# s-esposito/MonoGS

Measured on AMD Instinct MI355X. Metric: rasteriser fwd+bwd Mpix/s @1080p, higher is better.
Workload: dtype f32; 1 GPU; C5: 2000000 Gaussians, 1920x1080, fwd+bwd, seeded synthetic map (SURVEY.md 8d), one keyframe per GPU; gaussians=2000000, width=1920, height=1080, settle_steps=60, instance_count=device-side (capacity mode, overflow checked), parallelism=keyframe-per-gpu x1

## Files before the change

### monogs_amd/csrc/api.hip

```cpp
#include "common.h"

#include <stdarg.h>
#include <stdio.h>
#include <string.h>

namespace mgs {

static thread_local char g_err[512] = "";

void set_error(const char* fmt, ...) {
    va_list ap;
    va_start(ap, fmt);
    vsnprintf(g_err, sizeof(g_err), fmt, ap);
    va_end(ap);
}

static inline char* take(char*& p, size_t bytes) {
    char* r = p;
    p += align_up(bytes, 256);
    return r;
}

GeometryState GeometryState::carve(void* base, int P) {
    char* p = (char*)align_up((size_t)base, 256);
    GeometryState g;
    g.rec = (float*)take(p, (size_t)P * REC_FLOATS * sizeof(float));
    g.depth_key = (uint32_t*)take(p, (size_t)P * sizeof(uint32_t));
    g.depth_alt = (uint32_t*)take(p, (size_t)P * sizeof(uint32_t));
    g.iota = (uint32_t*)take(p, (size_t)P * sizeof(uint32_t));
    g.iota_alt = (uint32_t*)take(p, (size_t)P * sizeof(uint32_t));
    g.perm = (uint32_t*)take(p, (size_t)P * sizeof(uint32_t));
    g.point_offsets = (uint32_t*)take(p, (size_t)P * sizeof(uint32_t));
    g.scan_blocks = (uint32_t*)take(p, ((size_t)scan_nblocks(P) + 64) * sizeof(uint32_t));
    g.clamped = (uint8_t*)take(p, (size_t)P * 4);
    g.rect = (uint2*)take(p, (size_t)P * sizeof(uint2));
    g.rect_sorted = (uint2*)take(p, (size_t)P * sizeof(uint2));
    g.scan_status = (uint64_t*)take(p, (SCAN_SMALL_MAX_BLOCKS + 1) * sizeof(uint64_t));
    g.tile_hist = (uint32_t*)take(p, 4 * 256 * sizeof(uint32_t));
    g.sort_temp_bytes = radix_depth_temp_bytes((uint64_t)P);
    g.sort_temp = take(p, g.sort_temp_bytes);
    g.prepare = (unsigned long long*)take(p, 2 * sizeof(unsigned long long));
    g.end = p;
    return g;
}
size_t GeometryState::bytes(int P) {
    const GeometryState g = carve(nullptr, P);
    return (size_t)g.end + 256;
}

size_t ImageState::bytes(int W, int H) {
    const size_t HW = (size_t)W * H, nt = (size_t)tiles_x(W) * tiles_y(H);
    return align_up(HW * 4, 256) * 2 + align_up(nt * sizeof(uint2), 256) + 256;
}
ImageState ImageState::carve(void* base, int W, int H) {
    const size_t HW = (size_t)W * H, nt = (size_t)tiles_x(W) * tiles_y(H);
    char* p = (char*)align_up((size_t)base, 256);
    ImageState s;
    s.final_T = (float*)take(p, HW * 4);
    s.n_contrib = (uint32_t*)take(p, HW * 4);
    s.ranges = (uint2*)take(p, nt * sizeof(uint2));
    return s;
}

size_t BinningState::fwd_mask_rows(uint64_t R, int W, int H) {
    return (size_t)(R / 64) + (size_t)tiles_x(W) * tiles_y(H) + 1;
}
size_t BinningState::bytes(uint64_t R, int W, int H) {
    const size_t r = (size_t)(R ? R : 1);
    return align_up(r * 4, 256) * 4 + align_up(mgs::sort_temp_bytes(R, tile_bits(W, H)), 256) + 256 +
           align_up(fwd_mask_rows(R, W, H) * 4 * sizeof(unsigned long long), 256) + 256;
}
BinningState BinningState::carve(void* base, uint64_t R, int W, int H) {
    const size_t r = (size_t)(R ? R : 1);
    char* p = (char*)align_up((size_t)base, 256);
    BinningState b;
    b.keys_a = (uint32_t*)take(p, r * 4);
    b.keys_b = (uint32_t*)take(p, r * 4);
    b.vals_a = (uint32_t*)take(p, r * 4);
    b.vals_b = (uint32_t*)take(p, r * 4);
    const bool in_b = radix_result_in_b(tile_bits(W, H));
    b.keys_sorted = in_b ? b.keys_b : b.keys_a;
    b.vals_sorted = in_b ? b.vals_b : b.vals_a;
    b.sort_temp_bytes = mgs::sort_temp_bytes(R, tile_bits(W, H));
    b.sort_temp = take(p, b.sort_temp_bytes);
    b.count = (uint32_t*)take(p, 2 * sizeof(uint32_t));
    b.fwd_masks = (unsigned long long*)take(p, fwd_mask_rows(R, W, H) * 4 * sizeof(unsigned long long));
    return b;
}

struct StageTimer {
    hipStream_t s;
    bool on;
    hipEvent_t ev[10];
    int n = 0;
    StageTimer(hipStream_t s_, bool on_) : s(s_), on(on_) {
        if (on) for (auto& e : ev) (void)hipEventCreate(&e);
    }
    ~StageTimer() {
        if (on) for (auto& e : ev) (void)hipEventDestroy(e);
    }
    void mark() {
        if (on && n < 10) (void)hipEventRecord(ev[n++], s);
    }
    float ms(int i) {
        float t = 0.f;
        if (on && i + 1 < n) (void)hipEventElapsedTime(&t, ev[i], ev[i + 1]);
        return t;
    }
    void sync() {
        if (on && n) (void)hipEventSynchronize(ev[n - 1]);
    }
};

static int check_cam(const mgs_camera* cam) {
    if (!cam) { set_error("camera is NULL"); return 1; }
    if (cam->image_width <= 0 || cam->image_height <= 0) { set_error("image size must be positive"); return 1; }
    if (!cam->bg || !cam->viewmatrix || !cam->projmatrix || !cam->projmatrix_raw || !cam->campos) {
        set_error("camera tensors (bg, viewmatrix, projmatrix, projmatrix_raw, campos) must be non-NULL");
        return 1;
    }
    return 0;
}

static hipEvent_t g_dbg_fwd_events[2] = {nullptr, nullptr}, g_dbg_bwd_events[2] = {nullptr, nullptr};

static int check_map_size(int32_t P) {
    if (P > MGS_MAX_GAUSSIANS) {
        set_error("P exceeds MGS_MAX_GAUSSIANS (2^26 - 1): the gradient-line offset of the blend backward is 32-bit");
        return 1;
    }
    return 0;
}

}

using namespace mgs;

extern "C" {

int mgs_abi_version(void) { return MGS_ABI_VERSION; }
int mgs_binning_path(int32_t P, int32_t W, int32_t H) { return binning_path(P, W, H); }
const char* mgs_last_error(void) { return g_err; }

size_t mgs_geometry_bytes(int32_t P) { return GeometryState::bytes(P < 0 ? 0 : P); }
size_t mgs_image_bytes(int32_t W, int32_t H) { return ImageState::bytes(W, H); }
size_t mgs_binning_bytes(uint64_t R, int32_t W, int32_t H) { return BinningState::bytes(R, W, H); }
size_t mgs_backward_bytes(int32_t P) {
    return (size_t)(P < 0 ? 0 : P) * GRAD_FLOATS * sizeof(float) + (size_t)(TAU_SLOTS + 1) * 16 * sizeof(float) + 256;
}
float* mgs_backward_tau(void* backward_scratch, int32_t P) { return backward_tau_out(backward_scratch, P < 0 ? 0 : P); }

int mgs_forward_preprocess(const mgs_camera* cam, int32_t P, const float* means3D, const float* shs,
                           const float* colors_precomp, const float* opacities, const float* scales,
                           const float* rotations, const float* cov3D_precomp, void* geometry, int32_t* radii,
                           void* prepare_backward, uint64_t* num_rendered, const uint32_t* prev_status,
                           uint32_t* prev_status_out, mgs_timing* timing, void* stream) {
    if (check_cam(cam)) return 1;
    if (P < 0) { set_error("P must be >= 0"); return 1; }
    if (check_map_size(P)) return 1;
    if (num_rendered) *num_rendered = 0;
    if (prev_status_out) *prev_status_out = 0;
    if (P == 0) {
        if (prev_status && prev_status_out) {
            MGS_HIP(hipMemcpyAsync(prev_status_out, prev_status, sizeof(uint32_t), hipMemcpyDeviceToHost, (hipStream_t)stream));
            MGS_HIP(hipStreamSynchronize((hipStream_t)stream));
        }
        return 0;
    }
    if (!means3D || !opacities || !geometry || !radii) { set_error("means3D, opacities, geometry, radii must be non-NULL"); return 1; }
    if ((shs == nullptr) == (colors_precomp == nullptr)) {
        set_error("Please provide excatly one of either SHs or precomputed colors!");
        return 1;
    }
    const bool have_sr = scales != nullptr || rotations != nullptr;
    if ((have_sr && (!scales || !rotations || cov3D_precomp)) || (!have_sr && !cov3D_precomp)) {
        set_error("Please provide exactly one of either scale/rotation pair or precomputed 3D covariance!");
        return 1;
    }
    if (shs && (cam->sh_degree < 0 || cam->sh_degree > 3 || cam->sh_coeffs < (cam->sh_degree + 1) * (cam->sh_degree + 1))) {
        set_error("sh_degree must be 0..3 and shs must hold at least (degree+1)^2 coefficients");
        return 1;
    }
    hipStream_t s = (hipStream_t)stream;
    GeometryState g = GeometryState::carve(geometry, P);
    StageTimer tm(s, timing != nullptr);
    tm.mark();
    if (int rc = launch_preprocess_forward(*cam, P, means3D, shs, colors_precomp, opacities, scales, rotations,
                                           cov3D_precomp, g, radii,
                                           prepare_backward ? backward_grad_acc(prepare_backward) : nullptr, s)) return rc;
    tm.mark();
    const bool exclusive = (cam->flags & MGS_FLAG_EXCLUSIVE_DEVICE) != 0;
    const bool per_tile = binning_path(P, cam->image_width, cam->image_height) != 0;
    if (per_tile) {
        tm.mark();
        if (int rc = launch_scan(g, P, s, exclusive, g.rect)) return rc;
    } else {
        if (int rc = launch_depth_sort(g, P, depth_sort_payload(P, cam->image_width, cam->image_height), s, exclusive)) return rc;
        tm.mark();
        if (int rc = launch_scan(g, P, s, exclusive, g.rect_sorted)) return rc;
    }
    tm.mark();
    if (num_rendered) {
        uint32_t total = 0, sort_errors[RADIX_ERROR_WORDS] = {0, 0, 0, 0};
        MGS_HIP(hipMemcpyAsync(&total, g.scan_blocks + scan_nblocks(P), sizeof(uint32_t), hipMemcpyDeviceToHost, s));
        MGS_HIP(hipMemcpyAsync(sort_errors, radix_depth_error_flag(g.sort_temp, (uint64_t)P), sizeof(sort_errors),
                               hipMemcpyDeviceToHost, s));
        if (prev_status && prev_status_out)
            MGS_HIP(hipMemcpyAsync(prev_status_out, prev_status, sizeof(uint32_t), hipMemcpyDeviceToHost, s));
        MGS_HIP(hipStreamSynchronize(s));
        if (sort_errors[0] | sort_errors[1] | sort_errors[2] | sort_errors[3]) { set_error("depth sort: a look-back spin timed out (results invalid)"); return 3; }
        *num_rendered = total;
    }
    if (timing) {
        if (!num_rendered) MGS_HIP(hipStreamSynchronize(s));
        timing->preprocess_ms = tm.ms(0);
        timing->depth_sort_ms = per_tile ? 0.f : tm.ms(1);
        timing->scan_ms = tm.ms(2);
    }
    return 0;
}

static int g_opt_tile_sort_fused = 1;

static int forward_render_impl(const mgs_camera* cam, int32_t P, uint64_t R, bool capacity, void* geometry,
                               void* binning, void* image, float* out_color, float* out_depth, float* out_opacity,
                               int32_t* n_touched, uint32_t* overflow, mgs_timing* timing, void* stream) {
    if (check_cam(cam)) return 1;
    if (P < 0) { set_error("P must be >= 0"); return 1; }
    if (check_map_size(P)) return 1;
    if (!image || !out_color || !out_depth || !out_opacity) { set_error("image scratch and outputs must be non-NULL"); return 1; }
    if (P > 0 && (!geometry || !n_touched)) { set_error("geometry and n_touched must be non-NULL"); return 1; }
    if (R > 0 && !binning) { set_error("binning scratch is NULL"); return 1; }
    if (R >= (1ull << 32)) { set_error("num_rendered exceeds 2^32-1"); return 1; }
    if (P == 0) R = 0;
    hipStream_t s = (hipStream_t)stream;
    const int W = cam->image_width, H = cam->image_height;
    GeometryState g = GeometryState::carve(geometry, P);
    ImageState img = ImageState::carve(image, W, H);
    BinningState b = BinningState::carve(binning, R, W, H);
    const uint32_t* n_dev = nullptr;
    StageTimer tm(s, timing != nullptr);
    const bool cap = capacity && binning;
    if (cap) n_dev = b.count;
    const bool per_tile = binning_path(P, W, H) != 0;
    tm.mark();
    if (int rc = launch_duplicate(*cam, P, g, b, capacity ? R : (R > 0 ? 0xFFFFFFFFull : 0ull), n_touched, img, R,
                                  tile_bits(W, H), cap ? b.count : nullptr, overflow, s, per_tile)) return rc;
    tm.mark();
    if (int rc = launch_sort(g, b, R, tile_bits(W, H), s, n_dev, (cam->flags & MGS_FLAG_EXCLUSIVE_DEVICE) != 0, img.ranges,
                             per_tile)) return rc;
    const uint32_t* sort_err = R > 0 ? radix_error_flag(b.sort_temp, R, tile_bits(W, H)) : nullptr;
    const bool sort_tiles = per_tile && R > 0;
    const TileSortArgs ts = sort_tiles ? tile_sort_args(*cam, g, b, R, n_dev) : TileSortArgs{};
    const bool fused = sort_tiles && g_opt_tile_sort_fused != 0;
    if (sort_tiles && !fused)
        if (int rc = launch_tile_depth_sort(*cam, ts, img, sort_err, s)) return rc;
    tm.mark();
    if (g_dbg_fwd_events[0]) MGS_HIP(hipEventRecord(g_dbg_fwd_events[0], s));
    if (int rc = launch_blend_forward(*cam, g, b, img, out_color, out_depth, out_opacity, n_touched, sort_err, overflow,
                                      fused ? &ts : nullptr, P, s)) return rc;
    if (g_dbg_fwd_events[1]) MGS_HIP(hipEventRecord(g_dbg_fwd_events[1], s));
    tm.mark();
    if (timing) {
        tm.sync();
        timing->duplicate_ms = tm.ms(0);
        timing->sort_ms = tm.ms(1);
        timing->ranges_ms = 0.f;
        timing->blend_fwd_ms = tm.ms(2);
    }
    return 0;
}

int mgs_forward_render(const mgs_camera* cam, int32_t P, uint64_t R, void* geometry, void* binning, void* image,
                       float* out_color, float* out_depth, float* out_opacity, int32_t* n_touched,
                       uint32_t* status, mgs_timing* timing, void* stream) {
    return forward_render_impl(cam, P, R, false, geometry, binning, image, out_color, out_depth, out_opacity, n_touched,
                               status, timing, stream);
}

int mgs_forward_render_capacity(const mgs_camera* cam, int32_t P, uint64_t capacity, void* geometry, void* binning,
                                void* image, float* out_color, float* out_depth, float* out_opacity,
                                int32_t* n_touched, uint32_t* overflow, mgs_timing* timing, void* stream) {
    if (capacity == 0) { set_error("capacity must be > 0"); return 1; }
    return forward_render_impl(cam, P, capacity, true, geometry, binning, image, out_color, out_depth, out_opacity,
                               n_touched, overflow, timing, stream);
}

int mgs_forward_capacity(const mgs_camera* cam, int32_t P, const float* means3D, const float* shs,
                         const float* colors_precomp, const float* opacities, const float* scales, const float* rotations,
                         const float* cov3D_precomp, void* geometry, int32_t* radii, void* prepare_backward,
                         uint64_t capacity, void* binning, void* image, float* out_color, float* out_depth,
                         float* out_opacity, int32_t* n_touched, uint32_t* overflow, mgs_timing* timing, void* stream) {
    if (int rc = mgs_forward_preprocess(cam, P, means3D, shs, colors_precomp, opacities, scales, rotations, cov3D_precomp,
                                        geometry, radii, prepare_backward, nullptr, nullptr, nullptr, timing, stream)) return rc;
    return mgs_forward_render_capacity(cam, P, capacity, geometry, binning, image, out_color, out_depth, out_opacity,
                                       n_touched, overflow, timing, stream);
}

int mgs_backward(const mgs_camera* cam, int32_t P, uint64_t R, const float* means3D, const float* shs,
                 const float* colors_precomp, const float* opacities, const float* scales, const float* rotations,
                 const float* cov3D_precomp, const int32_t* radii, const void* geometry, const void* binning,
                 const void* image, const float* dL_dcolor, const float* dL_ddepth, const float* out_color,
                 const float* out_depth, float* dL_dmeans2D, float* dL_dcolors, float* dL_dopacity, float* dL_dmeans3D, float* dL_dcov3D, float* dL_dsh,
                 float* dL_dscales, float* dL_drotations, float* dL_dtau, void* backward_scratch,
                 int32_t scratch_prepared, mgs_timing* timing, void* stream) {
    if (check_cam(cam)) return 1;
    if (P < 0) { set_error("P must be >= 0"); return 1; }
    if (check_map_size(P)) return 1;
    hipStream_t s = (hipStream_t)stream;
    if (P == 0) {
        if (dL_dtau) MGS_HIP(zero_fill(dL_dtau, 6 * sizeof(float), s));
        return 0;
    }
    if (!means3D || !opacities || !radii || !geometry || !image || !dL_dcolor || !dL_ddepth || !backward_scratch) {
        set_error("means3D, opacities, radii, geometry, image, dL_dcolor, dL_ddepth, backward_scratch must be non-NULL");
        return 1;
    }
    if (R > 0 && !binning) { set_error("binning scratch is NULL"); return 1; }
    const int W = cam->image_width, H = cam->image_height;
    GeometryState g = GeometryState::carve(const_cast<void*>(geometry), P);
    ImageState img = ImageState::carve(const_cast<void*>(image), W, H);
    BinningState b = BinningState::carve(const_cast<void*>(binning), R, W, H);
    float* grad_acc = backward_grad_acc(backward_scratch);
    StageTimer tm(s, timing != nullptr);
    float* tau_part = (dL_dtau && (P + 255) / 256 > TAU_DIRECT_MAX_BLOCKS) ? backward_tau_part(backward_scratch, P) : nullptr;
    if (scratch_prepared) {
        if (dL_dtau && dL_dtau != backward_tau_out(backward_scratch, P)) {
            set_error("scratch_prepared: dL_dtau must be mgs_backward_tau(backward_scratch, P)");
            return 1;
        }
    } else {
        MGS_HIP(zero_fill2(grad_acc, (size_t)P * GRAD_FLOATS * sizeof(float) + (tau_part ? (size_t)TAU_SLOTS * 16 * sizeof(float) : 0),
                           dL_dtau, 6 * sizeof(float), s));
    }
    tm.mark();
    if (R > 0) {
        const bool pose_only = !dL_dcolors && !dL_dopacity && !dL_dsh && !shs;
        if (g_dbg_bwd_events[0]) MGS_HIP(hipEventRecord(g_dbg_bwd_events[0], s));
        if (int rc = launch_blend_backward(*cam, g, b, img, dL_dcolor, dL_ddepth, out_color, out_depth, grad_acc, pose_only, R, s)) return rc;
        if (g_dbg_bwd_events[1]) MGS_HIP(hipEventRecord(g_dbg_bwd_events[1], s));
    }
    tm.mark();
    GeomBackwardArgs a;
    a.means3D = means3D; a.shs = shs; a.colors_precomp = colors_precomp; a.opacities = opacities;
    a.scales = scales; a.rotations = rotations; a.cov3D_precomp = cov3D_precomp; a.radii = radii;
    a.grad_acc = grad_acc;
    a.dL_dmeans2D = dL_dmeans2D; a.dL_dcolors = dL_dcolors; a.dL_dopacity = dL_dopacity;
    a.dL_dmeans3D = dL_dmeans3D; a.dL_dcov3D = dL_dcov3D; a.dL_dsh = dL_dsh; a.dL_dscales = dL_dscales;
    a.dL_drotations = dL_drotations; a.dL_dtau = dL_dtau; a.tau_part = tau_part;
    if (int rc = launch_geom_backward(*cam, P, g, a, s)) return rc;
    tm.mark();
    if (timing) {
        tm.sync();
        timing->blend_bwd_ms = tm.ms(0);
        timing->geom_bwd_ms = tm.ms(1);
    }
    return 0;
}

int mgs_debug_blend_stats(const mgs_camera* cam, int32_t P, uint64_t R, const void* geometry, const void* binning,
                           const void* image, uint64_t* stats_dev, void* stream) {
    if (check_cam(cam)) return 1;
    if (!geometry || !image || !stats_dev || (R > 0 && !binning)) { set_error("bad arguments"); return 1; }
    hipStream_t s = (hipStream_t)stream;
    MGS_HIP(zero_fill(stats_dev, MGS_BLEND_STATS_WORDS * sizeof(uint64_t), s));
    if (P == 0 || R == 0) return 0;
    const int W = cam->image_width, H = cam->image_height;
    GeometryState g = GeometryState::carve(const_cast<void*>(geometry), P);
    ImageState img = ImageState::carve(const_cast<void*>(image), W, H);
    BinningState b = BinningState::carve(const_cast<void*>(binning), R, W, H);
    return launch_blend_backward_stats(*cam, g, b, img, (unsigned long long*)stats_dev, s);
}

int mgs_debug_blend_mask_stats(const mgs_camera* cam, int32_t P, uint64_t R, const void* geometry, const void* binning,
                               const void* image, uint64_t* stats_dev, void* stream) {
    if (check_cam(cam)) return 1;
    if (!geometry || !image || !stats_dev || (R > 0 && !binning)) { set_error("bad arguments"); return 1; }
    hipStream_t s = (hipStream_t)stream;
    MGS_HIP(zero_fill(stats_dev, MGS_BLEND_MASK_STATS_WORDS * sizeof(uint64_t), s));
    if (P == 0 || R == 0) return 0;
    const int W = cam->image_width, H = cam->image_height;
    GeometryState g = GeometryState::carve(const_cast<void*>(geometry), P);
    ImageState img = ImageState::carve(const_cast<void*>(image), W, H);
    BinningState b = BinningState::carve(const_cast<void*>(binning), R, W, H);
    return launch_blend_mask_stats(*cam, g, b, img, (unsigned long long*)stats_dev, s);
}

int mgs_debug_valu_ceiling(float* out, int32_t iters, void* stream) {
    if (!out || iters < 1) { set_error("mgs_debug_valu_ceiling: bad arguments"); return 1; }
    return launch_valu_ceiling(out, iters, (hipStream_t)stream);
}

int mgs_debug_last_backward_split(void) { return g_dbg_last_bwd_split; }

int mgs_debug_set_radix_spin_limit(uint32_t limit) { return set_radix_spin_limit(limit); }

int mgs_debug_set_blend_events(void* fwd_start, void* fwd_end, void* bwd_start, void* bwd_end) {
    if ((fwd_start == nullptr) != (fwd_end == nullptr) || (bwd_start == nullptr) != (bwd_end == nullptr)) {
        set_error("mgs_debug_set_blend_events: a pair is both events or neither");
        return 1;
    }
    g_dbg_fwd_events[0] = (hipEvent_t)fwd_start; g_dbg_fwd_events[1] = (hipEvent_t)fwd_end;
    g_dbg_bwd_events[0] = (hipEvent_t)bwd_start; g_dbg_bwd_events[1] = (hipEvent_t)bwd_end;
    return 0;
}

static int g_opt_debug_sort_exclusive = 0;
size_t mgs_debug_sort_temp_bytes(uint64_t n, int32_t bits) { return radix_temp_bytes(n, bits); }
int mgs_debug_sort_pairs(uint32_t* keys, uint32_t* vals, uint32_t* keys_alt, uint32_t* vals_alt, uint64_t n, int32_t bits,
                         void* temp, void* stream) {
    if (bits < 1 || bits > 32 || (n && (!keys || !vals || !keys_alt || !vals_alt || !temp))) {
        set_error("mgs_debug_sort_pairs: bad arguments");
        return 1;
    }
    if (n == 0) return 0;
    hipStream_t s = (hipStream_t)stream;
    if (int rc = radix_sort_pairs(keys, vals, keys_alt, vals_alt, n, bits, temp, s, nullptr, false, nullptr, nullptr, nullptr, false,
                                  g_opt_debug_sort_exclusive != 0))
        return rc;
    if (radix_result_in_b(bits)) {
        MGS_HIP(hipMemcpyAsync(keys, keys_alt, n * 4, hipMemcpyDeviceToDevice, s));
        MGS_HIP(hipMemcpyAsync(vals, vals_alt, n * 4, hipMemcpyDeviceToDevice, s));
    }
    uint32_t err[RADIX_ERROR_WORDS];
    MGS_HIP(hipMemcpyAsync(err, radix_error_flag(temp, n, bits), sizeof(err), hipMemcpyDeviceToHost, s));
    MGS_HIP(hipStreamSynchronize(s));
    if (err[0] | err[1] | err[2] | err[3]) { set_error("mgs_debug_sort_pairs: a look-back spin timed out"); return 2; }
    return 0;
}

int mgs_debug_set_option(const char* name, int64_t value) {
    if (name && !strcmp(name, "radix_scanned")) { g_opt_radix_scanned = (int)value; return 0; }
    if (name && !strcmp(name, "radix_ballot_rank")) { g_opt_radix_ballot_rank = (int)value; return 0; }
    if (name && !strcmp(name, "radix_xcd_band")) { g_opt_radix_xcd_band = (int)value; return 0; }
    if (name && !strcmp(name, "debug_sort_exclusive")) { g_opt_debug_sort_exclusive = (int)value; return 0; }
    if (name && !strcmp(name, "dup_slot_major")) { g_opt_dup_slot_major = (int)value; return 0; }
    if (name && !strcmp(name, "blend_bwd_transposed")) {
        g_opt_blend_bwd_transposed = value < 0 ? 2 : (int)value;
        g_opt_blend_bwd_transposed_set = value >= 0;
        return 0;
    }
    if (name && !strcmp(name, "blend_bwd_split")) { g_opt_blend_bwd_split = value < 0 ? -1 : (int)value; return 0; }
    if (name && !strcmp(name, "blend_bwd_split_min")) { g_opt_blend_bwd_split_min = value < 0 ? 4 : (int)value; return 0; }
    if (name && !strcmp(name, "blend_bwd_split_frac")) { g_opt_blend_bwd_split_frac = value < 0 ? 32 : (int)value; return 0; }
    if (name && !strcmp(name, "scan_small")) { g_opt_scan_small = (int)value; return 0; }
    if (name && !strcmp(name, "tile_sort_fused")) { g_opt_tile_sort_fused = value < 0 ? 1 : (int)value; return 0; }
    if (name && !strcmp(name, "knn_grid_min")) { g_opt_knn_grid_min = value > 0x7FFFFFFF ? 0x7FFFFFFF : (int)value; return 0; }
    set_error("mgs_debug_set_option: unknown option");
    return 1;
}

int mgs_mark_visible(int32_t P, const float* means3D, const float* viewmatrix, const float* projmatrix,
                     uint8_t* visible, void* stream) {
    (void)projmatrix;
    if (P < 0 || (P > 0 && (!means3D || !viewmatrix || !visible))) { set_error("bad arguments"); return 1; }
    return launch_mark_visible(P, means3D, viewmatrix, visible, (hipStream_t)stream);
}

size_t mgs_knn_scratch_bytes(int32_t P) { return knn_scratch_bytes(P); }

int mgs_dist2_knn(int32_t P, const float* points, float* out, void* scratch, void* stream) {
    if (P < 0 || (P > 0 && (!points || !out))) { set_error("bad arguments"); return 1; }
    return launch_knn(P, points, out, scratch, (hipStream_t)stream);
}

}
```

### monogs_amd/csrc/binning.hip

```cpp
#include "common.h"
#include "tile_sort.h"


namespace mgs {

constexpr int SCAN_THREADS = 256;
__device__ __forceinline__ int scan_nblocks_dev(int P) { return (P + SCAN_ITEMS - 1) / SCAN_ITEMS; }
constexpr int SCAN_PER_THREAD = SCAN_ITEMS / SCAN_THREADS;

__device__ __forceinline__ uint32_t wave_incl_scan(uint32_t v, int) { return wave_incl_scan_dpp(v); }

__device__ __forceinline__ uint32_t block_excl_scan(uint32_t v, uint32_t& total, uint32_t* smem ) {
    const int lane = threadIdx.x & 63, wv = threadIdx.x >> 6;
    const uint32_t incl = wave_incl_scan(v, lane);
    if (lane == 63) smem[wv] = incl;
    __syncthreads();
    uint32_t base = 0;
    for (int w = 0; w < wv; ++w) base += smem[w];
    total = smem[0] + smem[1] + smem[2] + smem[3];
    __syncthreads();
    return base + incl - v;
}

__device__ __forceinline__ uint32_t scan_block_rows(const uint2* __restrict__ rects, int n, int cbase, int lane, int wv,
                                                    uint32_t (&incl)[SCAN_PER_THREAD], uint32_t* smem ) {
    uint32_t v[SCAN_PER_THREAD];
#pragma unroll
    for (int i = 0; i < SCAN_PER_THREAD; ++i) {
        const int idx = cbase + i * WAVE + lane;
        const uint32_t wh = idx < n ? rects[idx].y : 0u;
        v[i] = (wh & 0xFFFFu) * (wh >> 16);
    }
    uint32_t run = 0;
#pragma unroll
    for (int i = 0; i < SCAN_PER_THREAD; ++i) {
        const uint32_t sc = wave_incl_scan_dpp(v[i]);
        incl[i] = run + sc;
        run += (uint32_t)__builtin_amdgcn_readlane((int)sc, 63);
    }
    if (lane == 0) smem[wv] = run;
    __syncthreads();
    uint32_t wbase = 0;
    for (int w = 0; w < wv; ++w) wbase += smem[w];
    const uint32_t total = (smem[0] + smem[1]) + (smem[2] + smem[3]);
#pragma unroll
    for (int i = 0; i < SCAN_PER_THREAD; ++i) incl[i] += wbase;
    return total;
}

__global__ void __launch_bounds__(SCAN_THREADS) scan_local_kernel(const uint2* __restrict__ rects, uint32_t* out,
                                                                  uint32_t* block_sums, int n) {
    __shared__ uint32_t smem[8];
    const int lane = threadIdx.x & 63, wv = threadIdx.x >> 6;
    const int cbase = blockIdx.x * SCAN_ITEMS + wv * (SCAN_PER_THREAD * WAVE);
    uint32_t incl[SCAN_PER_THREAD];
    const uint32_t total = scan_block_rows(rects, n, cbase, lane, wv, incl, smem);
#pragma unroll
    for (int i = 0; i < SCAN_PER_THREAD; ++i) {
        const int idx = cbase + i * WAVE + lane;
        if (idx < n) out[idx] = incl[i];
    }
    if (threadIdx.x == 0) block_sums[blockIdx.x] = total;
}

__global__ void __launch_bounds__(SCAN_THREADS) scan_blocks_kernel(uint32_t* block_sums, int nblocks) {
    __shared__ uint32_t smem[8];
    uint32_t carry = 0;
    for (int start = 0; start < nblocks; start += SCAN_THREADS) {
        const int i = start + threadIdx.x;
        const uint32_t v = i < nblocks ? block_sums[i] : 0u;
        uint32_t total;
        const uint32_t ex = block_excl_scan(v, total, smem);
        if (i < nblocks) block_sums[i] = carry + ex;
        carry += total;
    }
    if (threadIdx.x == 0) block_sums[nblocks] = carry;
}

constexpr uint32_t SCAN_SPIN_LIMIT = 1u << 22;
__global__ void __launch_bounds__(SCAN_THREADS) scan_small_kernel(const uint2* __restrict__ rects, uint32_t* out,
                                                                  uint32_t* block_sums, uint64_t* status, int n, int nb,
                                                                  uint32_t* err, int ticketed) {
    __shared__ uint32_t smem[8];
    __shared__ uint32_t s_prefix, s_bid;
    const int lane = threadIdx.x & 63, wv = threadIdx.x >> 6;
    int bid = (int)blockIdx.x;
    if (ticketed) {
        if (threadIdx.x == 0) s_bid = atomicAdd((uint32_t*)(status + SCAN_SMALL_MAX_BLOCKS), 1u);
        __syncthreads();
        bid = (int)s_bid;
    }
    const int cbase = bid * SCAN_ITEMS + wv * (SCAN_PER_THREAD * WAVE);
    uint32_t incl[SCAN_PER_THREAD];
    const uint32_t total = scan_block_rows(rects, n, cbase, lane, wv, incl, smem);
    if (threadIdx.x == 0)
        __hip_atomic_store(status + bid, (1ull << 63) | (uint64_t)total, __ATOMIC_RELAXED, __HIP_MEMORY_SCOPE_AGENT);
    if (threadIdx.x < WAVE) {
        uint32_t before = 0;
        if ((int)threadIdx.x < bid) {
            uint64_t w = 0;
            uint32_t spins = 0;
            while (true) {
                w = __hip_atomic_load(status + threadIdx.x, __ATOMIC_RELAXED, __HIP_MEMORY_SCOPE_AGENT);
                if (w >> 63) break;
                if (++spins > SCAN_SPIN_LIMIT) { atomicExch(err, 1u); break; }
                __builtin_amdgcn_s_sleep(1);
            }
            before = (uint32_t)w;
        }
#pragma unroll
        for (int o = 32; o > 0; o >>= 1) before += __shfl_xor(before, o, 64);
        if (threadIdx.x == 0) s_prefix = before;
    }
    __syncthreads();
#pragma unroll
    for (int i = 0; i < SCAN_PER_THREAD; ++i) {
        const int idx = cbase + i * WAVE + lane;
        if (idx < n) out[idx] = incl[i] + s_prefix;
    }
    if (threadIdx.x == 0 && bid == nb - 1) block_sums[nb] = s_prefix + total;
}
int g_opt_scan_small = -1;
bool scan_is_small(int P) { return g_opt_scan_small != 0 && scan_nblocks(P) <= SCAN_SMALL_MAX_BLOCKS; }


int launch_scan(const GeometryState& g, int P, hipStream_t s, bool exclusive, const uint2* rects) {
    if (P == 0) return 0;
    const int nb = scan_nblocks(P);
    if (scan_is_small(P)) {
        hipLaunchKernelGGL(scan_small_kernel, dim3(nb), dim3(SCAN_THREADS), 0, s, rects, g.point_offsets, g.scan_blocks,
                           g.scan_status, P, nb, const_cast<uint32_t*>(radix_depth_error_flag(g.sort_temp, (uint64_t)P)),
                           exclusive ? 0 : 1);
        MGS_HIP(hipGetLastError());
        return 0;
    }
    hipLaunchKernelGGL(scan_local_kernel, dim3(nb), dim3(SCAN_THREADS), 0, s, rects, g.point_offsets,
                       g.scan_blocks, P);
    hipLaunchKernelGGL(scan_blocks_kernel, dim3(1), dim3(SCAN_THREADS), 0, s, g.scan_blocks, nb);
    MGS_HIP(hipGetLastError());
    return 0;
}

__device__ __forceinline__ void dup_pair(uint32_t gidx, const uint32_t* __restrict__ depth_key, int lo, uint32_t& val,
                                         uint32_t& kfield) {
    val = gidx; kfield = 0u;
    if (depth_key) {
        const uint32_t k = depth_key[gidx];
        const uint32_t d = k == 0xFFFFFFFFu ? DEPTH_KEY_NARROW : min(k - DEPTH_KEY_SUB, DEPTH_KEY_NARROW);
        kfield = d >> lo;
        if (lo) val |= (d & ((1u << lo) - 1u)) << (32 - lo);
    }
}
__global__ void __launch_bounds__(256) duplicate_kernel(int P, const uint2* __restrict__ rects,
                                                        const uint32_t* __restrict__ perm,
                                                        const uint32_t* __restrict__ depth_key, int tshift, int lo,
                                                        const uint32_t* __restrict__ offsets ,
                                                        const uint32_t* __restrict__ block_sums ,
                                                        uint32_t* keys,
                                                        uint32_t* vals, int gx, int gy, uint32_t r_cap,
                                                        int32_t* __restrict__ n_touched, uint2* __restrict__ ranges,
                                                        int ntiles, uint32_t* __restrict__ zero_ptr, size_t zero_words,
                                                        uint32_t* __restrict__ count, uint32_t* __restrict__ overflow,
                                                        const uint32_t* __restrict__ depth_err, int offsets_global,
                                                        uint32_t* __restrict__ hist , int hist_passes,
                                                        int n_threads , int slot_major,
                                                        unsigned long long* __restrict__ prepare ) {
    const int i = blockIdx.x * 256 + threadIdx.x;
    if (i == 0 && prepare) {
        prepare[1] = prepare[0];
        prepare[0] = 0ull;
    }
    const int lane = threadIdx.x & 63;
    grid_zero(zero_ptr, zero_words, (size_t)n_threads, 256);
    const bool depth_bad = depth_err && radix_failed(depth_err) != 0u;
    if (i == 0 && count) {
        const uint32_t R = (P > 0 && !depth_bad) ? block_sums[scan_nblocks_dev(P)] : 0u;
        count[0] = min(R, r_cap);
        count[1] = R > r_cap ? 1u : 0u;
    }
    if (i == 0 && overflow)
        overflow[0] = (count ? count[1] : 0u) | (depth_bad ? (uint32_t)MGS_STATUS_DEPTH_SORT_TIMEOUT : 0u);
    if (i < ntiles) ranges[i] = make_uint2(0xFFFFFFFFu, 0u);
    if (i < P) n_touched[i] = 0;
    uint32_t idx = 0, nt = 0, off = 0, kf = 0;
    int x0 = 0, y0 = 0, x1 = 0;
    if (i < P) {
        dup_pair(perm ? perm[i] : (uint32_t)i, depth_key, lo, idx, kf);
        const uint2 r = rects[i];
        const int w = (int)(r.y & 0xFFFFu), h = (int)(r.y >> 16);
        nt = (uint32_t)(w * h);
        x0 = (int)(r.x & 0xFFFFu); y0 = (int)(r.x >> 16); x1 = x0 + w;
    }
    if (depth_bad) nt = 0;
    if (nt) off = i == 0 ? 0u : offsets[i - 1] + (offsets_global ? 0u : block_sums[(i - 1) / SCAN_ITEMS]);
    __shared__ uint32_t s_own[4][WAVE];
    __shared__ uint32_t s_idx[4][WAVE], s_off[4][WAVE], s_kf[4][WAVE];
    __shared__ int s_x0[4][WAVE], s_y0[4][WAVE], s_w[4][WAVE];
    __shared__ uint32_t s_hist[2][256];
    if (hist) {
        s_hist[0][threadIdx.x] = 0u; s_hist[1][threadIdx.x] = 0u;
        __syncthreads();
    }
    const int wv = threadIdx.x >> 6;
    if (slot_major) {
        const uint32_t R_all = (P > 0 && !depth_bad) ? block_sums[scan_nblocks_dev(P)] : 0u;
        const uint32_t R_emit = min(R_all, r_cap);
        const uint32_t n_waves = (uint32_t)n_threads / WAVE;
        const uint32_t CH = (((R_emit + n_waves - 1u) / n_waves) + 63u) & ~63u;
        const uint32_t wave_id = (uint32_t)blockIdx.x * 4u + (uint32_t)wv;
        const uint64_t s0w = (uint64_t)wave_id * CH;
        const uint32_t s0 = s0w < (uint64_t)R_emit ? (uint32_t)s0w : R_emit, s1 = (uint64_t)s0 + CH < (uint64_t)R_emit ? s0 + CH : R_emit;
        auto incl = [&](uint32_t k) { return offsets[k] + (offsets_global ? 0u : block_sums[k / SCAN_ITEMS]); };
        uint32_t g = 0;
        if (s0 < s1) {
            uint32_t lo = 0, hi = (uint32_t)P;
            while (hi - lo > 1u) {
                const uint32_t span = hi - lo, step = (span + 63u) / 64u;
                const uint32_t probe = lo + min(((uint32_t)lane + 1u) * step, span) - 1u;
                const unsigned long long above = __builtin_amdgcn_ballot_w64(incl(probe) > s0);
                const int k = __builtin_ctzll(above);
                const uint32_t pk = lo + min(((uint32_t)k + 1u) * step, span) - 1u;
                const uint32_t pk1 = k == 0 ? lo : lo + min((uint32_t)k * step, span);
                lo = pk1; hi = pk + 1u;
            }
            g = lo;
        }
        uint32_t sl = s0;
        while (sl < s1 && g < (uint32_t)P) {
            const uint32_t gi = g + (uint32_t)lane;
            const bool valid = gi < (uint32_t)P;
            uint32_t inc = 0, ntg = 0, idg = 0, kfg = 0;
            int gx0 = 0, gy0 = 0, gw = 1;
            if (valid) {
                inc = incl(gi);
                const uint2 r = rects[gi];
                gw = (int)(r.y & 0xFFFFu);
                ntg = (uint32_t)(gw * (int)(r.y >> 16));
                gx0 = (int)(r.x & 0xFFFFu); gy0 = (int)(r.x >> 16);
                dup_pair(perm ? perm[gi] : gi, depth_key, lo, idg, kfg);
            }
            const uint32_t exc = inc - ntg;
            uint32_t Eg = valid ? inc : 0u;
#pragma unroll
            for (int o2 = 32; o2 > 0; o2 >>= 1) Eg = max(Eg, (uint32_t)__shfl_xor((int)Eg, o2, 64));
            __builtin_amdgcn_wave_barrier();
            s_idx[wv][lane] = idg; s_kf[wv][lane] = kfg; s_off[wv][lane] = exc; s_x0[wv][lane] = gx0; s_y0[wv][lane] = gy0; s_w[wv][lane] = max(gw, 1);
            const uint32_t e = min(s1, Eg);
            const uint32_t cb0 = sl & ~63u;
            const unsigned long long before = __builtin_amdgcn_ballot_w64(ntg != 0u && exc < cb0);
            uint32_t carry = before ? 64u - (uint32_t)__builtin_clzll(before) : 0u;
            for (uint32_t cb = cb0; cb < e; cb += WAVE) {
                __builtin_amdgcn_wave_barrier();
                s_own[wv][lane] = 0u;
                __builtin_amdgcn_wave_barrier();
                if (ntg != 0u && exc >= cb && exc < cb + WAVE) s_own[wv][exc - cb] = (uint32_t)lane + 1u;
                __builtin_amdgcn_wave_barrier();
                uint32_t m = s_own[wv][lane];
#define MGS_DPP_MAX(ctrl, row_mask) m = max(m, (uint32_t)__builtin_amdgcn_update_dpp(0, (int)m, ctrl, row_mask, 0xf, false))
                MGS_DPP_MAX(0x111, 0xf); MGS_DPP_MAX(0x112, 0xf); MGS_DPP_MAX(0x114, 0xf); MGS_DPP_MAX(0x118, 0xf);
                MGS_DPP_MAX(0x142, 0xa); MGS_DPP_MAX(0x143, 0xc);
#undef MGS_DPP_MAX
                const uint32_t owner = max(m, carry);
                carry = (uint32_t)__builtin_amdgcn_readlane((int)owner, 63);
                const uint32_t o = cb + lane;
                if (owner != 0u && o >= sl && o < e) {
                    const uint32_t L = owner - 1u;
                    const uint32_t t = o - s_off[wv][L];
                    const uint32_t w = (uint32_t)s_w[wv][L];
                    const uint32_t yy = t / w, xx = t - yy * w;
                    const uint32_t tid = (uint32_t)((s_y0[wv][L] + (int)yy) * gx + s_x0[wv][L] + (int)xx);
                    const uint32_t key = (tid << tshift) | s_kf[wv][L];
                    keys[o] = key;
                    vals[o] = s_idx[wv][L];
                    if (hist) {
                        atomicAdd(&s_hist[0][(key >> tshift) & 0xFFu], 1u);
                        if (hist_passes > 1) {
                            const uint32_t d1 = (key >> (tshift + 8)) & 0xFFu;
                            const uint32_t lead = (uint32_t)__builtin_amdgcn_readfirstlane((int)d1);
                            const unsigned long long same = __builtin_amdgcn_ballot_w64(d1 == lead);
                            if (d1 != lead) atomicAdd(&s_hist[1][d1], 1u);
                            else if (lane == (int)__builtin_ctzll(same)) atomicAdd(&s_hist[1][lead], (uint32_t)__popcll(same));
                        }
                    }
                }
            }
            sl = max(sl, e);
            if (Eg <= sl) g += WAVE;
        }
        if (hist) {
            __syncthreads();
            const uint32_t c0 = s_hist[0][threadIdx.x], c1 = s_hist[1][threadIdx.x];
            if (c0) atomicAdd(hist + threadIdx.x, c0);
            if (c1) atomicAdd(hist + 256 + threadIdx.x, c1);
        }
        return;
    }
    s_idx[wv][lane] = idx; s_kf[wv][lane] = kf; s_off[wv][lane] = off; s_x0[wv][lane] = x0; s_y0[wv][lane] = y0; s_w[wv][lane] = max(x1 - x0, 1);
    const unsigned long long live = __builtin_amdgcn_ballot_w64(nt != 0);
    if (live == 0ull && !hist) return;
    const int first = live ? __builtin_ctzll(live) : 0, lastl = live ? 63 - __builtin_clzll(live) : 0;
    const uint32_t S = live ? (uint32_t)__builtin_amdgcn_readlane((int)off, first) : 0u;
    const uint32_t E = live ? (uint32_t)__builtin_amdgcn_readlane((int)(off + nt), lastl) : 0u;
    uint32_t carry = 0;
    for (uint32_t cb = S & ~63u; cb < E; cb += WAVE) {
        __builtin_amdgcn_wave_barrier();
        s_own[wv][lane] = 0u;
        __builtin_amdgcn_wave_barrier();
        if (nt != 0 && off >= cb && off < cb + WAVE) s_own[wv][off - cb] = (uint32_t)lane + 1u;
        __builtin_amdgcn_wave_barrier();
        uint32_t m = s_own[wv][lane];
#define MGS_DPP_MAX(ctrl, row_mask) m = max(m, (uint32_t)__builtin_amdgcn_update_dpp(0, (int)m, ctrl, row_mask, 0xf, false))
        MGS_DPP_MAX(0x111, 0xf); MGS_DPP_MAX(0x112, 0xf); MGS_DPP_MAX(0x114, 0xf); MGS_DPP_MAX(0x118, 0xf);
        MGS_DPP_MAX(0x142, 0xa); MGS_DPP_MAX(0x143, 0xc);
#undef MGS_DPP_MAX
        const uint32_t owner = max(m, carry);
        carry = (uint32_t)__builtin_amdgcn_readlane((int)owner, 63);
        const uint32_t o = cb + lane;
        if (owner != 0u && o < E && o < r_cap) {
            const uint32_t L = owner - 1u;
            const uint32_t t = o - s_off[wv][L];
            const uint32_t w = (uint32_t)s_w[wv][L];
            const uint32_t yy = t / w, xx = t - yy * w;
            const uint32_t tid = (uint32_t)((s_y0[wv][L] + (int)yy) * gx + s_x0[wv][L] + (int)xx);
            const uint32_t key = (tid << tshift) | s_kf[wv][L];
            keys[o] = key;
            vals[o] = s_idx[wv][L];
            if (hist) {
                atomicAdd(&s_hist[0][(key >> tshift) & 0xFFu], 1u);
                if (hist_passes > 1) {
                    const uint32_t d1 = (key >> (tshift + 8)) & 0xFFu;
                    const uint32_t lead = (uint32_t)__builtin_amdgcn_readfirstlane((int)d1);
                    const unsigned long long same = __builtin_amdgcn_ballot_w64(d1 == lead);
                    if (d1 != lead) atomicAdd(&s_hist[1][d1], 1u);
                    else if (lane == (int)__builtin_ctzll(same)) atomicAdd(&s_hist[1][lead], (uint32_t)__popcll(same));
                }
            }
        }
    }
    if (hist) {
        __syncthreads();
        const uint32_t c0 = s_hist[0][threadIdx.x], c1 = s_hist[1][threadIdx.x];
        if (c0) atomicAdd(hist + threadIdx.x, c0);
        if (c1) atomicAdd(hist + 256 + threadIdx.x, c1);
    }
}

constexpr uint64_t DUP_SLOT_MAJOR_MIN = 768ull * 1024;
int g_opt_dup_slot_major = -1;

int launch_duplicate(const mgs_camera& cam, int P, const GeometryState& g, const BinningState& b, uint64_t r_cap,
                     int32_t* n_touched, const ImageState& img, uint64_t sort_n, int sort_bits, uint32_t* count,
                     uint32_t* overflow, hipStream_t s, bool per_tile) {
    const uint32_t* depth_err = P > 0 ? radix_depth_error_flag(g.sort_temp, (uint64_t)P) : nullptr;
    const int ntiles = tiles_x(cam.image_width) * tiles_y(cam.image_height);
    int n = P > ntiles ? P : ntiles;
    if (n == 0) return 0;
    const bool slot_major = P > 0 && g_opt_dup_slot_major != 0 &&
                            (g_opt_dup_slot_major > 0 || (sort_n >= DUP_SLOT_MAJOR_MIN && sort_n >= 6ull * (uint64_t)P));
    if (slot_major) {
        const uint64_t want = sort_n / 8;
        if (want > (uint64_t)n) n = (int)(want > 0x3FFFFFFFull ? 0x3FFFFFFFull : want);
    }
    const int n_threads = (n + 255) / 256 * 256;
    uint32_t* zero_ptr = nullptr;
    size_t zero_words = 0;
    if (sort_n > 0) radix_zero_region(b.sort_temp, sort_n, sort_bits, &zero_ptr, &zero_words);
    const bool count_digits = P > 0 && sort_bits <= 16 && radix_wants_hist(sort_n);
    const int tb = tile_bits(cam.image_width, cam.image_height);
    hipLaunchKernelGGL(duplicate_kernel, dim3(n_threads / 256), dim3(256), 0, s, P, per_tile ? g.rect : g.rect_sorted,
                       per_tile ? nullptr : g.perm, per_tile ? g.depth_key : nullptr, per_tile ? 32 - tb : 0,
                       per_tile ? tile_depth_lo_bits(tb) : 0, g.point_offsets,
                       g.scan_blocks, b.keys_a, b.vals_a, tiles_x(cam.image_width), tiles_y(cam.image_height),
                       (uint32_t)(r_cap > 0xFFFFFFFFull ? 0xFFFFFFFFull : r_cap), n_touched, img.ranges, ntiles, zero_ptr,
                       zero_words, count, overflow, depth_err,
                       (P > 0 && scan_is_small(P)) ? 1 : 0,
                       count_digits ? g.tile_hist : nullptr, (sort_bits + 7) / 8, n_threads, slot_major ? 1 : 0,
                       P > 0 ? g.prepare : nullptr);
    MGS_HIP(hipGetLastError());
    return 0;
}

size_t sort_temp_bytes(uint64_t n, int bits) { return radix_temp_bytes(n, bits); }

int launch_depth_sort(const GeometryState& g, int P, bool payload, hipStream_t s, bool exclusive) {
    return radix_sort_depth(g.depth_key, g.depth_alt, g.iota, g.iota_alt, g.rect, payload, g.perm, g.rect_sorted, (uint64_t)P,
                            g.sort_temp, s, true, exclusive);
}

int launch_sort(const GeometryState& g, const BinningState& b, uint64_t R, int bits, hipStream_t s, const uint32_t* n_dev,
                bool exclusive, uint2* ranges, bool per_tile) {
    if (R == 0) return 0;
    const bool counted = bits <= 16 && radix_wants_hist(R) && g.tile_hist != nullptr;
    return radix_sort_pairs(b.keys_a, b.vals_a, b.keys_b, b.vals_b, R, bits, b.sort_temp, s, n_dev, true, nullptr, nullptr,
                            counted ? g.tile_hist : nullptr, false, exclusive, ranges, per_tile ? 32 - bits : 0);
}

TileSortArgs tile_sort_args(const mgs_camera& cam, const GeometryState& g, const BinningState& b, uint64_t R,
                            const uint32_t* n_dev) {
    TileSortArgs ts;
    ts.keys = b.keys_sorted;
    ts.vals = b.vals_sorted;
    ts.keys_alt = b.keys_sorted == b.keys_a ? b.keys_b : b.keys_a;
    ts.vals_alt = b.vals_sorted == b.vals_a ? b.vals_b : b.vals_a;
    ts.depth_key = g.depth_key;
    ts.n_dev = n_dev;
    ts.n_cap = (uint32_t)R;
    ts.tb = tile_bits(cam.image_width, cam.image_height);
    return ts;
}

__global__ void __launch_bounds__(TDS_THREADS) tile_depth_sort_kernel(TileSortArgs ts, const uint2* __restrict__ ranges,
                                                                       int ntiles, const uint32_t* __restrict__ sort_err) {
    __shared__ uint32_t s_k[TDS_CAP], s_v[TDS_CAP];
    __shared__ uint32_t s_cnt[TDS_WAVES][TDS_RADIX];
    __shared__ uint32_t s_wsum[TDS_WAVES], s_red[2 * TDS_WAVES];
    const int tile = blockIdx.x;
    if (tile >= ntiles) return;
    tile_depth_sort(ts, ranges[tile], sort_err && radix_failed(sort_err) != 0u, TdsLds{s_k, s_v, s_cnt, s_wsum, s_red});
}

int launch_tile_depth_sort(const mgs_camera& cam, const TileSortArgs& ts, const ImageState& img, const uint32_t* sort_err,
                           hipStream_t s) {
    const int ntiles = tiles_x(cam.image_width) * tiles_y(cam.image_height);
    hipLaunchKernelGGL(tile_depth_sort_kernel, dim3(ntiles), dim3(TDS_THREADS), 0, s, ts, img.ranges, ntiles, sort_err);
    MGS_HIP(hipGetLastError());
    return 0;
}


}
```

### monogs_amd/csrc/common.h

```cpp
#pragma once

#include <hip/hip_runtime.h>
#include <stdint.h>
#include <stddef.h>

#include "../../include/monogs_raster.h"

namespace mgs {

constexpr int TILE = MGS_TILE;
constexpr int WAVE = 64;
constexpr int SUB = 8;
constexpr int REC_FLOATS = 16;
constexpr int GRAD_FLOATS = 16;

enum : int {
    R_X = 0, R_Y = 1, R_EX = 2, R_EY = 3,
    R_CA = 4, R_CB = 5, R_CC = 6, R_OPAC = 7,
    R_R = 8, R_G = 9, R_B = 10, R_DEPTH = 11,
    R_NA = 12, R_NB = 13, R_NC = 14, R_RADIUS = 15
};
enum : int {
    G_SX = 0, G_SY = 1, G_SXX = 2, G_SXY = 3, G_SYY = 4, G_SH = 5,
    G_DR = 6, G_DG = 7, G_DB = 8, G_DDEPTH = 9
};

inline size_t align_up(size_t v, size_t a) { return (v + a - 1) / a * a; }

#if defined(__HIP_DEVICE_COMPILE__)
typedef const float __attribute__((address_space(4))) * const_float_p;
typedef const unsigned long long __attribute__((address_space(4))) * const_u64_p;
#define MGS_CONST(p) ((mgs::const_float_p)(p))
#define MGS_CONST_U64(p) ((mgs::const_u64_p)(p))
#else
typedef const float* const_float_p;
typedef const unsigned long long* const_u64_p;
#define MGS_CONST(p) (p)
#define MGS_CONST_U64(p) (p)
#endif

__device__ __forceinline__ uint32_t wave_incl_scan_dpp(uint32_t v) {
#define MGS_DPP_ADD(ctrl, row_mask) v += (uint32_t)__builtin_amdgcn_update_dpp(0, (int)v, ctrl, row_mask, 0xf, false)
    MGS_DPP_ADD(0x111, 0xf);
    MGS_DPP_ADD(0x112, 0xf);
    MGS_DPP_ADD(0x114, 0xf);
    MGS_DPP_ADD(0x118, 0xf);
    MGS_DPP_ADD(0x142, 0xa);
    MGS_DPP_ADD(0x143, 0xc);
#undef MGS_DPP_ADD
    return v;
}

__global__ static void zero_fill_kernel(uint32_t* __restrict__ p, size_t n_words, int vec) {
    const size_t i0 = (size_t)blockIdx.x * blockDim.x + threadIdx.x, stride = (size_t)gridDim.x * blockDim.x;
    if (vec) {
        uint4* q = reinterpret_cast<uint4*>(p);
        const size_t nv = n_words / 4;
        for (size_t i = i0; i < nv; i += stride) q[i] = make_uint4(0u, 0u, 0u, 0u);
        for (size_t i = nv * 4 + i0; i < n_words; i += stride) p[i] = 0u;
    } else {
        for (size_t i = i0; i < n_words; i += stride) p[i] = 0u;
    }
}
__device__ __forceinline__ void grid_zero(uint32_t* __restrict__ p, size_t n_words, size_t threads, int block) {
    const size_t i0 = (size_t)blockIdx.x * block + threadIdx.x, stride = threads;
    uint4* q = reinterpret_cast<uint4*>(p);
    const size_t nv = n_words / 4;
    for (size_t i = i0; i < nv; i += stride) q[i] = make_uint4(0u, 0u, 0u, 0u);
    for (size_t i = nv * 4 + i0; i < n_words; i += stride) p[i] = 0u;
}
__global__ static void zero_fill2_kernel(uint32_t* __restrict__ p, size_t n_words, uint32_t* __restrict__ p2, int n2) {
    grid_zero(p, n_words, (size_t)gridDim.x * 256, 256);
    if (blockIdx.x == 0 && (int)threadIdx.x < n2) p2[threadIdx.x] = 0u;
}
static inline hipError_t zero_fill2(void* ptr, size_t bytes, void* ptr2, size_t bytes2, hipStream_t s) {
    const size_t n_words = bytes / 4;
    size_t blocks = (n_words / 4 + 255) / 256;
    blocks = blocks < 1 ? 1 : (blocks > 4096 ? 4096 : blocks);
    hipLaunchKernelGGL(zero_fill2_kernel, dim3((unsigned)blocks), dim3(256), 0, s, (uint32_t*)ptr, n_words,
                       (uint32_t*)ptr2, ptr2 ? (int)(bytes2 / 4) : 0);
    return hipGetLastError();
}
static inline hipError_t zero_fill(void* ptr, size_t bytes, hipStream_t s) {
    if (bytes == 0) return hipSuccess;
    const size_t n_words = bytes / 4;
    const int vec = ((size_t)ptr % 16 == 0) ? 1 : 0;
    const size_t items = vec ? (n_words + 3) / 4 : n_words;
    size_t blocks = (items + 255) / 256;
    if (blocks > 4096) blocks = 4096;
    hipLaunchKernelGGL(zero_fill_kernel, dim3((unsigned)blocks), dim3(256), 0, s, (uint32_t*)ptr, n_words, vec);
    return hipGetLastError();
}

struct GeometryState {
    float* rec;
    uint32_t* depth_key;
    uint32_t* depth_alt;
    uint32_t* iota;
    uint32_t* iota_alt;
    uint32_t* perm;
    uint32_t* point_offsets;
    uint32_t* scan_blocks;
    uint8_t* clamped;
    uint2* rect;
    uint2* rect_sorted;
    uint64_t* scan_status;
    uint32_t* tile_hist;
    void* sort_temp;
    size_t sort_temp_bytes;
    unsigned long long* prepare;
    char* end;
    static size_t bytes(int P);
    static GeometryState carve(void* base, int P);
};
constexpr int SCAN_SMALL_MAX_BLOCKS = 64;

struct ImageState {
    float* final_T;
    uint32_t* n_contrib;
    uint2* ranges;
    static size_t bytes(int W, int H);
    static ImageState carve(void* base, int W, int H);
};

struct BinningState {
    uint32_t* keys_a;
    uint32_t* vals_a;
    uint32_t* keys_b;
    uint32_t* vals_b;
    uint32_t* keys_sorted;
    uint32_t* vals_sorted;
    void* sort_temp;
    size_t sort_temp_bytes;
    uint32_t* count;
    unsigned long long* fwd_masks;
    static size_t fwd_mask_rows(uint64_t R, int W, int H);
    static size_t bytes(uint64_t R, int W, int H);
    static BinningState carve(void* base, uint64_t R, int W, int H);
};

constexpr int SCAN_ITEMS = 2048;
inline int scan_nblocks(int P) { return (P + SCAN_ITEMS - 1) / SCAN_ITEMS; }

inline int tiles_x(int W) { return (W + TILE - 1) / TILE; }
inline int tiles_y(int H) { return (H + TILE - 1) / TILE; }
inline int tile_bits(int W, int H) {
    uint32_t n = (uint32_t)(tiles_x(W) * tiles_y(H));
    int b = 0;
    while ((1u << b) < n && b < 31) ++b;
    return b == 0 ? 1 : b;
}

constexpr uint32_t DEPTH_KEY_SUB = 0x3E4CCCCDu;
constexpr uint32_t DEPTH_KEY_NARROW = (1u << 27) - 1u;
__host__ __device__ inline int tile_depth_lo_bits(int tb) { return tb > 5 ? tb - 5 : 0; }
int binning_path(int P, int W, int H);

void set_error(const char* fmt, ...);
#define MGS_HIP(expr)                                                                     \
    do {                                                                                  \
        hipError_t _e = (expr);                                                           \
        if (_e != hipSuccess) {                                                           \
            mgs::set_error("%s failed: %s (%s:%d)", #expr, hipGetErrorString(_e), __FILE__, __LINE__); \
            return 2;                                                                     \
        }                                                                                 \
    } while (0)

struct StageTimer;

int launch_preprocess_forward(const mgs_camera& cam, int P, const float* means3D, const float* shs,
                              const float* colors_precomp, const float* opacities, const float* scales,
                              const float* rotations, const float* cov3D_precomp,
                              const GeometryState& g, int32_t* radii, float* prepare_grad_acc, hipStream_t s);
constexpr int TAU_SLOTS = 256;
inline float* backward_grad_acc(void* scratch) { return (float*)align_up((size_t)scratch, 256); }
inline float* backward_tau_part(void* scratch, int P) { return backward_grad_acc(scratch) + (size_t)P * GRAD_FLOATS; }
inline float* backward_tau_out(void* scratch, int P) { return backward_tau_part(scratch, P) + (size_t)TAU_SLOTS * 16; }
int launch_scan(const GeometryState& g, int P, hipStream_t s, bool exclusive, const uint2* rects);
int launch_duplicate(const mgs_camera& cam, int P, const GeometryState& g, const BinningState& b, uint64_t r_cap,
                     int32_t* n_touched, const ImageState& img, uint64_t sort_n, int sort_bits, uint32_t* count,
                     uint32_t* overflow, hipStream_t s, bool per_tile);
size_t sort_temp_bytes(uint64_t n, int bits);
size_t radix_temp_bytes(uint64_t n, int bits);
size_t radix_depth_temp_bytes(uint64_t n);
bool radix_result_in_b(int bits);
constexpr int RADIX_ERROR_WORDS = 4;
const uint32_t* radix_error_flag(void* temp, uint64_t n, int bits);
const uint32_t* radix_depth_error_flag(void* temp, uint64_t n);
__device__ __forceinline__ uint32_t radix_failed(const uint32_t* __restrict__ e) { return (e[0] | e[1]) | (e[2] | e[3]); }
void radix_zero_region(void* temp, uint64_t n, int bits, uint32_t** ptr, size_t* words);
void radix_depth_zero_region(void* temp, uint64_t n, uint32_t** ptr, size_t* words, bool header_only = false);
int radix_sort_pairs(uint32_t* ka, uint32_t* va, uint32_t* kb, uint32_t* vb, uint64_t n, int bits, void* temp,
                     hipStream_t s, const uint32_t* n_dev = nullptr, bool temp_zeroed = false,
                     const uint2* aux_in = nullptr, uint2* aux_out = nullptr,
                     const uint32_t* ext_hist = nullptr,
                     bool aux_empty_for_ones = false,
                     bool exclusive = false,
                     uint2* ranges = nullptr,
                     int key_shift = 0);
bool radix_wants_hist(uint64_t n);
bool radix_depth_payload(uint64_t n);
int radix_sort_depth(uint32_t* keys, uint32_t* key_b, uint32_t* val_a, uint32_t* val_b, void* rect, bool payload,
                     uint32_t* perm, uint2* rect_sorted, uint64_t n, void* temp, hipStream_t s, bool temp_zeroed,
                     bool exclusive = false);
inline bool depth_sort_payload(int P, int W, int H) { return radix_depth_payload((uint64_t)P) && tiles_x(W) <= 255 && tiles_y(H) <= 255; }
int launch_depth_sort(const GeometryState& g, int P, bool payload, hipStream_t s, bool exclusive = false);
int launch_sort(const GeometryState& g, const BinningState& b, uint64_t R, int bits, hipStream_t s,
                const uint32_t* n_dev = nullptr, bool exclusive = false, uint2* ranges = nullptr, bool per_tile = false);
struct TileSortArgs {
    uint32_t* keys;
    uint32_t* vals;
    uint32_t* keys_alt;
    uint32_t* vals_alt;
    const uint32_t* depth_key;
    const uint32_t* n_dev;
    uint32_t n_cap;
    int tb;
};
TileSortArgs tile_sort_args(const mgs_camera& cam, const GeometryState& g, const BinningState& b, uint64_t R,
                            const uint32_t* n_dev);
int launch_tile_depth_sort(const mgs_camera& cam, const TileSortArgs& ts, const ImageState& img, const uint32_t* sort_err,
                           hipStream_t s);
int set_radix_spin_limit(uint32_t limit);
extern bool g_opt_blend_bwd_transposed_set;
extern int g_dbg_last_bwd_split;
extern int g_opt_radix_ballot_rank, g_opt_radix_scanned, g_opt_radix_xcd_band, g_opt_knn_grid_min, g_opt_scan_small, g_opt_dup_slot_major, g_opt_blend_bwd_transposed, g_opt_blend_bwd_split, g_opt_blend_bwd_split_min, g_opt_blend_bwd_split_frac;
int launch_blend_forward(const mgs_camera& cam, const GeometryState& g, const BinningState& b,
                         const ImageState& img, float* out_color, float* out_depth, float* out_opacity,
                         int32_t* n_touched, const uint32_t* sort_err, uint32_t* status, const TileSortArgs* tile_sort,
                         int P, hipStream_t s);
int launch_blend_backward(const mgs_camera& cam, const GeometryState& g, const BinningState& b,
                          const ImageState& img, const float* dL_dcolor, const float* dL_ddepth, const float* out_color,
                          const float* out_depth, float* grad_acc, bool pose_only, uint64_t num_rendered, hipStream_t s);
int launch_blend_backward_stats(const mgs_camera& cam, const GeometryState& g, const BinningState& b,
                                const ImageState& img, unsigned long long* stats, hipStream_t s);
int launch_blend_mask_stats(const mgs_camera& cam, const GeometryState& g, const BinningState& b,
                            const ImageState& img, unsigned long long* stats, hipStream_t s);
int launch_valu_ceiling(float* out, int iters, hipStream_t s);
struct GeomBackwardArgs {
    const float *means3D, *shs, *colors_precomp, *opacities, *scales, *rotations, *cov3D_precomp;
    const int32_t* radii;
    const float* grad_acc;
    float *dL_dmeans2D, *dL_dcolors, *dL_dopacity, *dL_dmeans3D, *dL_dcov3D, *dL_dsh, *dL_dscales,
        *dL_drotations, *dL_dtau;
    float* tau_part;
};
constexpr int TAU_DIRECT_MAX_BLOCKS = 256;
int launch_geom_backward(const mgs_camera& cam, int P, const GeometryState& g, const GeomBackwardArgs& a,
                         hipStream_t s);
int launch_mark_visible(int P, const float* means3D, const float* viewmatrix, uint8_t* visible, hipStream_t s);
size_t knn_scratch_bytes(int P);
int launch_knn(int P, const float* points, float* out, void* scratch, hipStream_t s);

}
```

### monogs_amd/csrc/radix_sort.hip

```cpp
#include "common.h"

namespace mgs {

#ifdef RS_TRACE
__device__ uint64_t* g_rs_trace = nullptr;
#define RS_STAMP(k) do { if (g_rs_trace && threadIdx.x == 0) g_rs_trace[(size_t)blockIdx.x * 8 + (k)] = wall_clock64(); } while (0)
#define RS_DRAIN() asm volatile("s_waitcnt vmcnt(0) lgkmcnt(0)" ::: "memory")
__device__ uint64_t* g_rs_htrace = nullptr;
#define RS_HSTAMP(k) do { if (g_rs_htrace && threadIdx.x == 0) g_rs_htrace[(size_t)blockIdx.x * 4 + (k)] = wall_clock64(); } while (0)
#else
#define RS_HSTAMP(k)
#define RS_STAMP(k)
#define RS_DRAIN()
#endif

constexpr int RS_THREADS = 256;
constexpr int RS_WAVES = RS_THREADS / WAVE;
constexpr int RS_ITEMS = 16;
constexpr int RS_ITEMS_WIDE = 12;
constexpr int RS_ITEMS_MID = 8;
constexpr int RS_ITEMS_SMALL = 4;
constexpr uint64_t RS_ONE_SWEEP_MAX = 512ull * 1024;
static inline int rs_items(uint64_t n) {
    return n <= 192ull * 1024 ? RS_ITEMS_SMALL : (n <= RS_ONE_SWEEP_MAX ? RS_ITEMS_MID : RS_ITEMS);
}
constexpr int RS_MAX_RADIX = 512;
constexpr int RS_MAX_PASSES = 4;
constexpr uint64_t RS_FLAG_LOCAL = 1ull << 62;
constexpr uint64_t RS_FLAG_GLOBAL = 2ull << 62;
constexpr uint64_t RS_COUNT_MASK = (1ull << 62) - 1;
constexpr uint32_t RS_SPIN_LIMIT = 1u << 22;
__device__ uint32_t g_rs_spin_limit = RS_SPIN_LIMIT;
constexpr uint32_t RS_GROUP = 16;

constexpr uint32_t RS_DEPTH_SUB = DEPTH_KEY_SUB;
constexpr uint32_t RS_DEPTH_NARROW = DEPTH_KEY_NARROW;
__device__ __forceinline__ uint32_t rs_xf(uint32_t k, uint32_t sub) { return k == 0xFFFFFFFFu ? k : k - sub; }

int g_opt_radix_scanned = -1;
int g_opt_radix_ballot_rank = 0;
int g_opt_radix_xcd_band = 1;
constexpr uint64_t RS_SCANNED_MIN = 64ull * 1024;
static inline bool rs_scanned(uint64_t n) {
    if (g_opt_radix_scanned >= 0) return g_opt_radix_scanned == 1 && n > RS_SCANNED_MIN;
    return n > RS_ONE_SWEEP_MAX;
}

int binning_path(int P, int W, int H) {
    if (P <= 0) return 0;
    const bool large = g_opt_radix_scanned >= 0 ? g_opt_radix_scanned == 1 : (uint64_t)P > RS_ONE_SWEEP_MAX;
    const int tb = tile_bits(W, H);
    if (!large || tb > 16) return 0;
    return (uint64_t)P <= (1ull << (32 - tile_depth_lo_bits(tb))) ? 1 : 0;
}
static inline int rs_tile_items(uint64_t n, bool scanned) {
    if (!scanned) return rs_items(n);
    return n > 1024ull * RS_THREADS * RS_ITEMS ? RS_ITEMS_WIDE : RS_ITEMS;
}
static inline uint32_t rs_tiles(uint64_t n, bool scanned) {
    const uint64_t tile = (uint64_t)RS_THREADS * rs_tile_items(n, scanned);
    return (uint32_t)((n + tile - 1) / tile);
}
static inline uint32_t rs_tiles(uint64_t n) { return rs_tiles(n, rs_scanned(n)); }

struct RsPlan {
    int npasses;
    int shift[RS_MAX_PASSES];
    int db[RS_MAX_PASSES];
    int radix;
    uint32_t sub;
    bool depth;
};
static inline RsPlan rs_plan_plain(int bits) {
    RsPlan pl;
    pl.npasses = (bits + 7) / 8;
    for (int p = 0; p < RS_MAX_PASSES; ++p) { pl.shift[p] = 8 * p; pl.db[p] = 8; }
    pl.radix = 256; pl.sub = 0u; pl.depth = false;
    return pl;
}
static inline RsPlan rs_plan_depth() {
    RsPlan pl;
    pl.npasses = 4;
    for (int p = 0; p < 3; ++p) { pl.shift[p] = 9 * p; pl.db[p] = 9; }
    pl.shift[3] = 27; pl.db[3] = 8;
    pl.radix = 512; pl.sub = RS_DEPTH_SUB; pl.depth = true;
    return pl;
}

static inline RsPlan rs_plan_for_depth(uint64_t n) { return rs_scanned(n) ? rs_plan_depth() : rs_plan_plain(32); }

constexpr int RS_FAN_LOG = 2;
constexpr int RS_TOP_BATCH = 8;
constexpr int RS_MAX_LEVELS = 6;
struct RsTree {
    int levels;
    uint32_t rows[RS_MAX_LEVELS];
    uint32_t off[RS_MAX_LEVELS];
    uint32_t sum_rows;
};
static inline RsTree rs_tree(uint32_t tiles) {
    RsTree tr;
    tr.levels = 1; tr.rows[0] = tiles; tr.off[0] = 0; tr.sum_rows = 0;
    while (tr.rows[tr.levels - 1] > (uint32_t)RS_TOP_BATCH && tr.levels < RS_MAX_LEVELS) {
        tr.rows[tr.levels] = (tr.rows[tr.levels - 1] + (1u << RS_FAN_LOG) - 1u) >> RS_FAN_LOG;
        tr.off[tr.levels] = tr.sum_rows;
        tr.sum_rows += tr.rows[tr.levels];
        ++tr.levels;
    }
    return tr;
}

static inline size_t rs_status_rows(uint32_t tiles) { return (size_t)tiles + (tiles + RS_GROUP - 1) / RS_GROUP; }
struct RsTemp {
    uint32_t* hist;
    uint32_t* tickets;
    uint32_t* error;
    uint32_t* wide;
    uint64_t* status;
    uint32_t* sums;
    uint32_t* counts;
    size_t zero_bytes;
    size_t bytes;
};
static RsTemp rs_carve(void* temp, uint64_t n, const RsPlan& pl, bool scanned) {
    char* p = (char*)align_up((size_t)temp, 256);
    RsTemp t;
    t.hist = (uint32_t*)p;
    t.tickets = t.hist + RS_MAX_PASSES * pl.radix;
    t.error = t.tickets + RS_MAX_PASSES;
    t.wide = t.error + RS_MAX_PASSES;
    char* q = (char*)align_up((size_t)(t.wide + 1), 256);
    t.status = (uint64_t*)q;
    t.sums = (uint32_t*)q;
    const uint32_t tiles = rs_tiles(n, scanned);
    if (scanned) {
        const size_t sums_bytes = (size_t)pl.npasses * rs_tree(tiles).sum_rows * pl.radix * sizeof(uint32_t);
        t.counts = (uint32_t*)(q + sums_bytes);
        t.zero_bytes = (size_t)(q - p) + sums_bytes;
        t.bytes = t.zero_bytes + (size_t)tiles * pl.radix * sizeof(uint32_t);
    } else {
        t.counts = nullptr;
        t.zero_bytes = (size_t)(q - p) + (size_t)pl.npasses * rs_status_rows(tiles) * pl.radix * sizeof(uint64_t);
        t.bytes = t.zero_bytes;
    }
    return t;
}
static size_t rs_temp_bytes(uint64_t n, const RsPlan& pl) {
    if (n == 0) return 256;
    const size_t a = rs_carve(nullptr, n, pl, false).bytes;
    const size_t b = n > RS_SCANNED_MIN ? rs_carve(nullptr, n, pl, true).bytes : 0;
    return (a > b ? a : b) + 512;
}
size_t radix_temp_bytes(uint64_t n, int bits) { return rs_temp_bytes(n, rs_plan_plain(bits)); }
size_t radix_depth_temp_bytes(uint64_t n) {
    const size_t a = rs_temp_bytes(n, rs_plan_depth()), b = rs_temp_bytes(n, rs_plan_plain(32));
    return a > b ? a : b;
}


struct RsHistArgs {
    int npasses, radix;
    int shift[RS_MAX_PASSES], mask[RS_MAX_PASSES];
    uint32_t sub;
    uint32_t* wide;
};
__global__ void __launch_bounds__(RS_THREADS) rs_hist_kernel(const uint32_t* __restrict__ keys, uint32_t n,
                                                             const uint32_t* __restrict__ n_dev, RsHistArgs h,
                                                             uint32_t* __restrict__ hist) {
    __shared__ uint32_t lh[RS_WAVES][RS_MAX_PASSES * RS_MAX_RADIX];
    if (n_dev) n = min(n, n_dev[0]);
    const int words = h.npasses * h.radix;
    for (int w = 0; w < RS_WAVES; ++w)
        for (int i = threadIdx.x; i < words; i += RS_THREADS) lh[w][i] = 0;
    __syncthreads();
    const int wv = threadIdx.x >> 6;
    bool far = false;
    for (uint32_t i = blockIdx.x * RS_THREADS + threadIdx.x; i < n; i += gridDim.x * RS_THREADS) {
        const uint32_t k = keys[i], x = rs_xf(k, h.sub);
        far |= k != 0xFFFFFFFFu && x >= RS_DEPTH_NARROW;
        for (int p = 0; p < h.npasses; ++p) atomicAdd(&lh[wv][p * h.radix + ((x >> h.shift[p]) & h.mask[p])], 1u);
    }
    if (h.wide && far) atomicOr(h.wide, 1u);
    __syncthreads();
    for (int i = threadIdx.x; i < words; i += RS_THREADS) {
        uint32_t c = 0;
#pragma unroll
        for (int w = 0; w < RS_WAVES; ++w) c += lh[w][i];
        if (c) atomicAdd(hist + i, c);
    }
}

struct RsTreeArgs {
    int levels;
    uint32_t off[RS_MAX_LEVELS];
    uint32_t top_rows;
};
struct RsTileHistArgs {
    const uint32_t* keys;
    uint32_t n;
    const uint32_t* n_dev;
    int shift;
    uint32_t sub;
    uint32_t tiles;
    RsTreeArgs tr;
    uint32_t* counts;
    uint32_t* sums;
    uint32_t* wide;
    int detect;
    int only_if_wide;
};
template <int ITEMS, int TPW, int DB>
__global__ void __launch_bounds__(RS_THREADS * TPW) rs_tile_hist_kernel(RsTileHistArgs a) {
    static_assert(TPW == 1 || TPW == (1 << RS_FAN_LOG), "a workgroup counts one tile or one level-1 node");
    constexpr int RADIX = 1 << DB, DPT = RADIX / RS_THREADS, COPIES = 16 / DPT;
    constexpr uint32_t TILE_PAIRS = RS_THREADS * ITEMS;
    __shared__ uint32_t wh[TPW][COPIES][RADIX];
    const int t = threadIdx.x & (RS_THREADS - 1), q = threadIdx.x >> 8, wv = t >> 6, lane = t & 63;
    if (a.only_if_wide && a.wide[0] == 0u) return;
    RS_HSTAMP(0);
    const uint32_t n_live = a.n_dev ? min(a.n, a.n_dev[0]) : a.n;
    if (a.tr.levels > 1 && (uint64_t)blockIdx.x * TPW * TILE_PAIRS >= n_live) return;
    const uint32_t tile = blockIdx.x * TPW + q, tile_start = tile * TILE_PAIRS;
    const uint32_t tile_n = tile_start < n_live ? min(TILE_PAIRS, n_live - tile_start) : 0u;
    uint32_t k[ITEMS];
#pragma unroll
    for (int i = 0; i < ITEMS; ++i) {
        const uint32_t e = (uint32_t)i * RS_THREADS + t;
        k[i] = e < tile_n ? a.keys[tile_start + e] : 0xFFFFFFFFu;
    }
#pragma unroll
    for (int i = 0; i < COPIES; ++i)
#pragma unroll
        for (int j = 0; j < DPT; ++j) wh[q][i][t * DPT + j] = 0;
    __syncthreads();
    RS_DRAIN();
    RS_HSTAMP(1);
    uint32_t* mine = wh[q][wv * (COPIES / RS_WAVES) + (lane & (COPIES / RS_WAVES - 1))];
    bool far = false;
#pragma unroll
    for (int i = 0; i < ITEMS; ++i) {
        const uint32_t x = rs_xf(k[i], a.sub);
        far |= k[i] != 0xFFFFFFFFu && x >= RS_DEPTH_NARROW;
        if ((uint32_t)i * RS_THREADS + t < tile_n) atomicAdd(&mine[(x >> a.shift) & (RADIX - 1)], 1u);
    }
    if (a.detect && far) atomicOr(a.wide, 1u);
    __syncthreads();
    RS_HSTAMP(2);
    uint32_t c[DPT];
#pragma unroll
    for (int j = 0; j < DPT; ++j) {
        c[j] = 0;
#pragma unroll
        for (int i = 0; i < COPIES; ++i) c[j] += wh[q][i][t * DPT + j];
        if (tile < a.tiles) a.counts[(size_t)tile * RADIX + t * DPT + j] = c[j];
    }
    if (TPW == 1) {
#pragma unroll
        for (int j = 0; j < DPT; ++j)
            if (c[j])
                for (int l = 1; l < a.tr.levels; ++l)
                    atomicAdd(a.sums + ((size_t)a.tr.off[l] + (tile >> (RS_FAN_LOG * l))) * RADIX + t * DPT + j, c[j]);
    } else if (a.tr.levels > 1) {
        __syncthreads();
#pragma unroll
        for (int j = 0; j < DPT; ++j) wh[q][0][t * DPT + j] = c[j];
        __syncthreads();
        if (q == 0) {
#pragma unroll
            for (int j = 0; j < DPT; ++j) {
                uint32_t s1 = 0;
#pragma unroll
                for (int m = 0; m < TPW; ++m) s1 += wh[m][0][t * DPT + j];
                a.sums[((size_t)a.tr.off[1] + blockIdx.x) * RADIX + t * DPT + j] = s1;
                if (s1)
                    for (int l = 2; l < a.tr.levels; ++l)
                        atomicAdd(a.sums + ((size_t)a.tr.off[l] + (blockIdx.x >> (RS_FAN_LOG * (l - 1)))) * RADIX + t * DPT + j, s1);
            }
        }
    }
    RS_DRAIN();
    RS_HSTAMP(3);
}
template <int ITEMS, int DB>
static void rs_launch_tile_hist(const RsTileHistArgs& a, hipStream_t s) {
    if (a.tiles >= 1024u)
        hipLaunchKernelGGL((rs_tile_hist_kernel<ITEMS, 4, DB>), dim3((a.tiles + 3) / 4), dim3(RS_THREADS * 4), 0, s, a);
    else
        hipLaunchKernelGGL((rs_tile_hist_kernel<ITEMS, 1, DB>), dim3(a.tiles), dim3(RS_THREADS), 0, s, a);
}

struct RsPassArgs {
    const uint32_t* kin;
    const uint32_t* vin;
    const uint32_t* pin;
    uint32_t* kout;
    uint32_t* vout;
    uint32_t* pout;
    uint32_t* vfinal;
    uint32_t* kfinal;
    const uint2* aux_in;
    uint2* aux_out;
    int aux_skip_ones;
    uint32_t n;
    const uint32_t* n_dev;
    int shift;
    uint32_t sub;
    const uint32_t* hist;
    uint64_t* status;
    uint32_t tiles;
    uint32_t* ticket;
    uint32_t* error;
    int pass;
    int xcd_band;
    int last;
    int range_shift;
    int cond;
    const uint32_t* wide;
    uint2* ranges;
    const uint32_t* counts;
    const uint32_t* sums;
    RsTreeArgs tree;
};

template <int ITEMS>
__device__ __forceinline__ void rs_exchange(uint32_t* __restrict__ sbuf, const uint32_t (&slot)[ITEMS], uint32_t (&x)[ITEMS], int t) {
#pragma unroll
    for (int i = 0; i < ITEMS; ++i)
        if (slot[i] != 0xFFFFFFFFu) sbuf[slot[i]] = x[i];
    __syncthreads();
#pragma unroll
    for (int i = 0; i < ITEMS; ++i) x[i] = sbuf[min((uint32_t)i * RS_THREADS + (uint32_t)t, (uint32_t)(RS_THREADS * ITEMS - 1))];
}

template <int DPT>
__device__ __forceinline__ void rs_digit_bases(const uint32_t (&hcount)[DPT], uint32_t (&gdigit_base)[DPT], uint32_t* wsum, int lane, int wv) {
    uint32_t hsum = 0;
#pragma unroll
    for (int j = 0; j < DPT; ++j) hsum += hcount[j];
    const uint32_t hincl = wave_incl_scan_dpp(hsum);
    __syncthreads();
    if (lane == 63) wsum[wv] = hincl;
    __syncthreads();
    uint32_t hadd = 0;
    for (int w = 0; w < wv; ++w) hadd += wsum[w];
    uint32_t run = hadd + hincl - hsum;
#pragma unroll
    for (int j = 0; j < DPT; ++j) { gdigit_base[j] = run; run += hcount[j]; }
}

__device__ __forceinline__ bool rs_gather(const uint64_t* row, size_t stride, uint32_t cnt, uint32_t& pre, uint32_t& spins,
                                          uint32_t* err) {
    constexpr uint32_t G = RS_GROUP;
    for (uint32_t r0 = 0; r0 < cnt; r0 += G) {
        uint64_t w[G];
        bool ready;
        do {
#pragma unroll
            for (uint32_t q = 0; q < G; ++q) {
                const uint32_t r = r0 + q;
                w[q] = r < cnt ? __hip_atomic_load(row + (size_t)r * stride, __ATOMIC_RELAXED, __HIP_MEMORY_SCOPE_AGENT)
                                              : RS_FLAG_GLOBAL;
            }
            ready = true;
#pragma unroll
            for (uint32_t q = 0; q < G; ++q) ready &= (w[q] >> 62) != 0ull;
            if (!ready) {
                if (++spins > g_rs_spin_limit) { atomicExch(err, 1u); return false; }
                __builtin_amdgcn_s_sleep(1);
            }
        } while (!ready);
#pragma unroll
        for (uint32_t q = 0; q < G; ++q) pre += (uint32_t)(w[q] & RS_COUNT_MASK);
    }
    return true;
}

template <int ITEMS, int DB, bool SCANNED, bool PAYLOAD, bool BALLOT, bool VIDX>
__global__ void __launch_bounds__(RS_THREADS, (SCANNED && ITEMS == RS_ITEMS_WIDE && DB == 8 && !PAYLOAD) ? 7 : 1) rs_pass_kernel(RsPassArgs a) {
    constexpr int TILE_PAIRS = RS_THREADS * ITEMS;
    constexpr int RADIX = 1 << DB, DPT = RADIX / RS_THREADS;
    constexpr int SBUF = (SCANNED && 2 * RS_WAVES * RADIX > TILE_PAIRS) ? 2 * RS_WAVES * RADIX : TILE_PAIRS;
    __shared__ uint32_t wave_hist[RS_WAVES][RADIX];
    __shared__ uint32_t digit_base[RADIX];
    __shared__ uint32_t gbase[RADIX];
    __shared__ uint32_t sbuf[SBUF];
    __shared__ uint32_t wsum[RS_WAVES];
    __shared__ uint32_t s_tile;

    const int t = threadIdx.x, lane = t & 63, wv = t >> 6;
    const bool wide = a.wide ? a.wide[0] != 0u : false;
    if (a.cond == 2 && !wide) return;
    RS_STAMP(0);
    const bool final_pass = a.cond == 0 ? a.last != 0 : (a.cond == 1 ? !wide : true);
    if (!SCANNED) {
        uint32_t failed = 0;
        for (int q = 0; q < a.pass; ++q) failed |= a.error[q];
        if (failed) return;
    }
    const uint32_t n_live = a.n_dev ? min(a.n, a.n_dev[0]) : a.n;
    if (t == 0) {
        uint32_t id = blockIdx.x;
        if (a.xcd_band) {
            const uint32_t live = (n_live + (uint32_t)TILE_PAIRS - 1) / (uint32_t)TILE_PAIRS;
            const uint32_t q = live >> 3, r = live & 7u, x = id & 7u, j = id >> 3;
            id = j < q + (x < r ? 1u : 0u) ? x * q + min(x, r) + j : 0xFFFFFFFFu;
        }
        s_tile = (!SCANNED && a.ticket) ? atomicAdd(a.ticket, 1u) : id;
    }
#pragma unroll
    for (int w = 0; w < RS_WAVES; ++w)
#pragma unroll
        for (int j = 0; j < DPT; ++j) wave_hist[w][t * DPT + j] = 0;
    __syncthreads();
    const uint32_t tile = s_tile;
    if (tile == 0xFFFFFFFFu) return;
    const uint32_t tile_start = tile * (uint32_t)TILE_PAIRS;
    if (tile_start >= n_live) return;
    const uint32_t tile_n = min((uint32_t)TILE_PAIRS, n_live - tile_start);

    uint32_t hcount[DPT], before[DPT];
#pragma unroll
    for (int j = 0; j < DPT; ++j) hcount[j] = before[j] = 0;
    constexpr int R4 = RADIX / 4;
    uint4 lv[RS_MAX_LEVELS - 1][DPT], tv[RS_TOP_BATCH / RS_WAVES][DPT];
    uint32_t lw[RS_MAX_LEVELS - 1], tw[RS_TOP_BATCH / RS_WAVES], tb[RS_TOP_BATCH / RS_WAVES];
    const int levels = a.tree.levels;
    const uint32_t top_node = tile >> (RS_FAN_LOG * (levels - 1));
    const uint4* __restrict__ c4 = reinterpret_cast<const uint4*>(a.counts);
    const uint4* __restrict__ top4 = levels == 1 ? c4 : reinterpret_cast<const uint4*>(a.sums) + (size_t)a.tree.off[levels - 1] * R4;
    if (SCANNED) {
#pragma unroll
        for (int l = 0; l < RS_MAX_LEVELS - 1; ++l) {
            const bool have = l < levels - 1;
            const uint32_t node = tile >> (RS_FAN_LOG * l), first = node & ~3u, nb = node & 3u;
            const uint4* base = (l == 0 || !have) ? c4 : reinterpret_cast<const uint4*>(a.sums) + (size_t)a.tree.off[l] * R4;
            lw[l] = (have && (uint32_t)wv < nb) ? 1u : 0u;
#pragma unroll
            for (int j = 0; j < DPT; ++j) lv[l][j] = base[(size_t)(lw[l] ? first + (uint32_t)wv : 0u) * R4 + j * WAVE + lane];
        }
#pragma unroll
        for (int q = 0; q < RS_TOP_BATCH / RS_WAVES; ++q) {
            const uint32_t r = (uint32_t)wv + 4u * q;
            tw[q] = r < a.tree.top_rows ? 1u : 0u;
            tb[q] = r < top_node ? 1u : 0u;
#pragma unroll
            for (int j = 0; j < DPT; ++j) tv[q][j] = top4[(size_t)(tw[q] ? r : 0u) * R4 + j * WAVE + lane];
        }
    } else {
#pragma unroll
        for (int j = 0; j < DPT; ++j) hcount[j] = a.hist[t * DPT + j];
    }

    uint32_t key[ITEMS], val[ITEMS], rank[ITEMS], pay[PAYLOAD ? ITEMS : 1];
#pragma unroll
    for (int i = 0; i < ITEMS; ++i) {
        const uint32_t e = (uint32_t)wv * (ITEMS * WAVE) + (uint32_t)i * WAVE + lane;
        const bool valid = e < tile_n;
        key[i] = valid ? a.kin[tile_start + e] : 0xFFFFFFFFu;
        if constexpr (VIDX) val[i] = tile_start + e;
        else val[i] = valid ? a.vin[tile_start + e] : 0u;
        if constexpr (PAYLOAD) pay[i] = valid ? a.pin[tile_start + e] : 0u;
    }
    if (SCANNED) {
        uint4* part = reinterpret_cast<uint4*>(sbuf);
#pragma unroll
        for (int j = 0; j < DPT; ++j) {
            uint4 ab = make_uint4(0u, 0u, 0u, 0u), at = make_uint4(0u, 0u, 0u, 0u);
#pragma unroll
            for (int l = 0; l < RS_MAX_LEVELS - 1; ++l) {
                ab.x += lw[l] ? lv[l][j].x : 0u; ab.y += lw[l] ? lv[l][j].y : 0u; ab.z += lw[l] ? lv[l][j].z : 0u; ab.w += lw[l] ? lv[l][j].w : 0u;
            }
#pragma unroll
            for (int q = 0; q < RS_TOP_BATCH / RS_WAVES; ++q) {
                at.x += tw[q] ? tv[q][j].x : 0u; at.y += tw[q] ? tv[q][j].y : 0u; at.z += tw[q] ? tv[q][j].z : 0u; at.w += tw[q] ? tv[q][j].w : 0u;
                ab.x += tb[q] ? tv[q][j].x : 0u; ab.y += tb[q] ? tv[q][j].y : 0u; ab.z += tb[q] ? tv[q][j].z : 0u; ab.w += tb[q] ? tv[q][j].w : 0u;
            }
            for (uint32_t r0 = RS_TOP_BATCH; r0 < a.tree.top_rows; r0 += RS_TOP_BATCH)
#pragma unroll
                for (int q = 0; q < RS_TOP_BATCH / RS_WAVES; ++q) {
                    const uint32_t r = r0 + (uint32_t)wv + 4u * q;
                    if (r < a.tree.top_rows) {
                        const uint4 v = top4[(size_t)r * R4 + j * WAVE + lane];
                        at.x += v.x; at.y += v.y; at.z += v.z; at.w += v.w;
                        if (r < top_node) { ab.x += v.x; ab.y += v.y; ab.z += v.z; ab.w += v.w; }
                    }
                }
            part[(wv * 2 + 0) * R4 + j * WAVE + lane] = ab;
            part[(wv * 2 + 1) * R4 + j * WAVE + lane] = at;
        }
    }
    RS_DRAIN();
    RS_STAMP(1);
    if (!BALLOT) {
#pragma unroll
        for (int i = 0; i < ITEMS; ++i) {
            const uint32_t e = (uint32_t)wv * (ITEMS * WAVE) + (uint32_t)i * WAVE + lane;
            const uint32_t d = (rs_xf(key[i], a.sub) >> a.shift) & (RADIX - 1);
            rank[i] = 0;
            if (e < tile_n) rank[i] = __hip_atomic_fetch_add(&wave_hist[wv][d], 1u, __ATOMIC_RELAXED, __HIP_MEMORY_SCOPE_WORKGROUP);
        }
    } else {
        const unsigned long long lt_mask = (1ull << lane) - 1ull;
#pragma unroll
        for (int i = 0; i < ITEMS; ++i) {
            const uint32_t e = (uint32_t)wv * (ITEMS * WAVE) + (uint32_t)i * WAVE + lane;
            const bool valid = e < tile_n;
            const uint32_t d = (rs_xf(key[i], a.sub) >> a.shift) & (RADIX - 1);
            unsigned long long peers = __builtin_amdgcn_ballot_w64(valid);
#pragma unroll
            for (int b = 0; b < DB; ++b) {
                const bool bit = (d >> b) & 1u;
                const unsigned long long bm = __builtin_amdgcn_ballot_w64(valid && bit);
                peers &= bit ? bm : ~bm;
            }
            rank[i] = 0;
            if (valid) {
                const uint32_t prev = wave_hist[wv][d];
                rank[i] = prev + (uint32_t)__popcll(peers & lt_mask);
                if ((peers & lt_mask) == 0ull) wave_hist[wv][d] = prev + (uint32_t)__popcll(peers);
            }
        }
    }
    __syncthreads();
    if (SCANNED) {
#pragma unroll
        for (int j = 0; j < DPT; ++j)
#pragma unroll
            for (int w = 0; w < RS_WAVES; ++w) {
                before[j] += sbuf[(w * 2 + 0) * RADIX + t * DPT + j];
                hcount[j] += sbuf[(w * 2 + 1) * RADIX + t * DPT + j];
            }
    }
    RS_STAMP(2);

    uint32_t total[DPT], tsum = 0;
#pragma unroll
    for (int j = 0; j < DPT; ++j) {
        uint32_t run = 0;
#pragma unroll
        for (int w = 0; w < RS_WAVES; ++w) {
            const uint32_t c = wave_hist[w][t * DPT + j];
            wave_hist[w][t * DPT + j] = run;
            run += c;
        }
        total[j] = run;
        tsum += run;
    }
    const uint32_t incl = wave_incl_scan_dpp(tsum);
    if (lane == 63) wsum[wv] = incl;
    __syncthreads();
    uint32_t wadd = 0;
    for (int w = 0; w < wv; ++w) wadd += wsum[w];
    uint32_t dbase[DPT];
    {
        uint32_t run = wadd + incl - tsum;
#pragma unroll
        for (int j = 0; j < DPT; ++j) { dbase[j] = run; digit_base[t * DPT + j] = run; run += total[j]; }
    }
    uint32_t gdigit_base[DPT];
    if constexpr (SCANNED) {
        rs_digit_bases<DPT>(hcount, gdigit_base, wsum, lane, wv);
#pragma unroll
        for (int j = 0; j < DPT; ++j) gbase[t * DPT + j] = gdigit_base[j] + before[j] - dbase[j];
        __syncthreads();
    } else {
        static_assert(DPT == 1, "the one-sweep path ranks 256 digits");
        constexpr uint32_t G = RS_GROUP;
        const uint32_t live_tiles = (n_live + (uint32_t)TILE_PAIRS - 1) / (uint32_t)TILE_PAIRS;
        const uint32_t grp = tile / G, jin = tile % G;
        const uint32_t members = min(G, live_tiles - grp * G);
        uint64_t* gstat = a.status + (size_t)a.tiles * RADIX;
        rs_digit_bases<DPT>(hcount, gdigit_base, wsum, lane, wv);
        __hip_atomic_store(a.status + (size_t)tile * RADIX + t, RS_FLAG_LOCAL | (uint64_t)total[0], __ATOMIC_RELAXED,
                           __HIP_MEMORY_SCOPE_AGENT);
        uint32_t spins = 0, pre = 0, gpre = 0;
        bool ok = rs_gather(a.status + (size_t)grp * G * RADIX + t, RADIX, jin, pre, spins, a.error + a.pass);
        if (jin == members - 1)
            __hip_atomic_store(gstat + (size_t)grp * RADIX + t, RS_FLAG_GLOBAL | (uint64_t)(pre + total[0]), __ATOMIC_RELAXED,
                               __HIP_MEMORY_SCOPE_AGENT);
        if (ok) ok = rs_gather(gstat + t, RADIX, grp, gpre, spins, a.error + a.pass);
        gbase[t] = gdigit_base[0] + gpre + pre - dbase[0];
        __syncthreads();
    }

    RS_STAMP(3);
#pragma unroll
    for (int i = 0; i < ITEMS; ++i) {
        const uint32_t e = (uint32_t)wv * (ITEMS * WAVE) + (uint32_t)i * WAVE + lane;
        const uint32_t d = (rs_xf(key[i], a.sub) >> a.shift) & (RADIX - 1);
        rank[i] = e < tile_n ? digit_base[d] + wave_hist[wv][d] + rank[i] : 0xFFFFFFFFu;
    }
    rs_exchange<ITEMS>(sbuf, rank, key, t);
    __syncthreads();
    rs_exchange<ITEMS>(sbuf, rank, val, t);
    if constexpr (PAYLOAD) {
        __syncthreads();
        rs_exchange<ITEMS>(sbuf, rank, pay, t);
    }
    RS_STAMP(4);
    uint32_t g[ITEMS];
    bool live[ITEMS];
#pragma unroll
    for (int i = 0; i < ITEMS; ++i) {
        const uint32_t p = (uint32_t)i * RS_THREADS + t;
        live[i] = p < tile_n;
        g[i] = gbase[(rs_xf(key[i], a.sub) >> a.shift) & (RADIX - 1)] + p;
    }
    if (!final_pass) {
#pragma unroll
        for (int i = 0; i < ITEMS; ++i)
            if (live[i]) {
                a.kout[g[i]] = key[i];
                a.vout[g[i]] = val[i];
                if constexpr (PAYLOAD) a.pout[g[i]] = pay[i];
            }
        RS_STAMP(5); RS_DRAIN(); RS_STAMP(6); RS_STAMP(7);
        return;
    }
#pragma unroll
    for (int i = 0; i < ITEMS; ++i)
        if (live[i]) {
            if (a.kfinal) a.kfinal[g[i]] = key[i];
            a.vfinal[g[i]] = val[i];
        }
    if (a.ranges) {
        __shared__ uint32_t s_edge[RS_WAVES * ITEMS];
        if (lane == 63) {
#pragma unroll
            for (int i = 0; i < ITEMS; ++i) s_edge[wv * ITEMS + i] = key[i];
        }
        __syncthreads();
#pragma unroll
        for (int i = 0; i < ITEMS; ++i) {
            const uint32_t p = (uint32_t)i * RS_THREADS + t;
            uint32_t l = (uint32_t)__shfl_up((int)key[i], 1, 64);
            if (lane == 0) l = wv > 0 ? s_edge[(wv - 1) * ITEMS + i] : (i > 0 ? s_edge[(RS_WAVES - 1) * ITEMS + i - 1] : 0xFFFFFFFFu);
            const uint32_t kr = key[i] >> a.range_shift, lr = l >> a.range_shift;
            if (p < tile_n && (p == 0 || lr != kr)) {
                atomicMin(&a.ranges[kr].x, g[i]);
                if (p > 0)
                    atomicMax(&a.ranges[lr].y, gbase[(rs_xf(l, a.sub) >> a.shift) & (RADIX - 1)] + p);
            }
            if (p + 1 == tile_n) atomicMax(&a.ranges[kr].y, g[i] + 1u);
        }
    }
    RS_STAMP(5);
    RS_DRAIN();
    RS_STAMP(6);
    if (a.aux_out) {
        uint2* __restrict__ aout = a.aux_out;
        if constexpr (PAYLOAD) {
#pragma unroll
            for (int i = 0; i < ITEMS; ++i)
                if (live[i]) {
                    const uint32_t r = pay[i];
                    aout[g[i]] = key[i] == 0xFFFFFFFFu ? make_uint2(0u, 0u)
                                                       : make_uint2((r & 0xFFu) | ((r & 0xFF00u) << 8), ((r >> 16) & 0xFFu) | ((r >> 24) << 16));
                }
        } else {
            const uint2* __restrict__ ain = a.aux_in;
            uint2 r[ITEMS];
#pragma unroll
            for (int i = 0; i < ITEMS; ++i)
                r[i] = (live[i] && !(a.aux_skip_ones && key[i] == 0xFFFFFFFFu)) ? ain[val[i]] : make_uint2(0u, 0u);
#pragma unroll
            for (int i = 0; i < ITEMS; ++i)
                if (live[i]) aout[g[i]] = r[i];
        }
    }
    RS_DRAIN();
    RS_STAMP(7);
}


bool radix_result_in_b(int bits) { return (rs_plan_plain(bits).npasses & 1) != 0; }

const uint32_t* radix_error_flag(void* temp, uint64_t n, int bits) {
    return rs_carve(temp, n ? n : 1, rs_plan_plain(bits), rs_scanned(n ? n : 1)).error;
}
const uint32_t* radix_depth_error_flag(void* temp, uint64_t n) {
    return rs_carve(temp, n ? n : 1, rs_plan_for_depth(n ? n : 1), rs_scanned(n ? n : 1)).error;
}

void radix_zero_region(void* temp, uint64_t n, int bits, uint32_t** ptr, size_t* words) {
    const RsTemp t = rs_carve(temp, n ? n : 1, rs_plan_plain(bits), rs_scanned(n ? n : 1));
    *ptr = t.hist;
    *words = t.zero_bytes / 4;
}
void radix_depth_zero_region(void* temp, uint64_t n, uint32_t** ptr, size_t* words, bool header_only) {
    const RsTemp t = rs_carve(temp, n ? n : 1, rs_plan_for_depth(n ? n : 1), rs_scanned(n ? n : 1));
    *ptr = t.hist;
    *words = header_only ? (size_t)((char*)t.status - (char*)t.hist) / 4 : t.zero_bytes / 4;
}

bool radix_wants_hist(uint64_t n) { return n > 0 && !rs_scanned(n); }
bool radix_depth_payload(uint64_t n) { return n > 0 && rs_scanned(n); }

template <int ITEMS, int DB, bool SCANNED, bool PAYLOAD>
static void rs_launch_pass(const RsPassArgs& a, uint32_t tiles, bool ballot, hipStream_t s) {
    if (ballot && DB == 8 && !PAYLOAD && a.vin != nullptr)
        hipLaunchKernelGGL((rs_pass_kernel<ITEMS, 8, SCANNED, false, true, false>), dim3(tiles), dim3(RS_THREADS), 0, s, a);
    else if (a.vin == nullptr && (DB == 9 || !SCANNED))
        hipLaunchKernelGGL((rs_pass_kernel<ITEMS, DB, SCANNED, PAYLOAD, false, (DB == 9 || !SCANNED)>), dim3(tiles), dim3(RS_THREADS), 0, s, a);
    else
        hipLaunchKernelGGL((rs_pass_kernel<ITEMS, DB, SCANNED, PAYLOAD, false, false>), dim3(tiles), dim3(RS_THREADS), 0, s, a);
}
template <int DB, bool PAYLOAD>
static void rs_launch_pass_items(const RsPassArgs& a, int items, bool scanned, uint32_t tiles, bool ballot, hipStream_t s) {
    if (scanned) {
        if (items == RS_ITEMS_WIDE) rs_launch_pass<RS_ITEMS_WIDE, DB, true, PAYLOAD>(a, tiles, ballot, s);
        else rs_launch_pass<RS_ITEMS, DB, true, PAYLOAD>(a, tiles, ballot, s);
    } else if constexpr (!PAYLOAD && DB == 8) {
        if (items == RS_ITEMS_SMALL) rs_launch_pass<RS_ITEMS_SMALL, 8, false, false>(a, tiles, ballot, s);
        else if (items == RS_ITEMS_MID) rs_launch_pass<RS_ITEMS_MID, 8, false, false>(a, tiles, ballot, s);
        else rs_launch_pass<RS_ITEMS, 8, false, false>(a, tiles, ballot, s);
    }
}

struct RsBuffers {
    uint2* ranges;
    uint32_t *ka, *va, *pa;
    bool va_is_index;
    uint32_t *kb, *vb, *pb;
    uint32_t *kfinal, *vfinal;
    const uint2* aux_in;
    uint2* aux_out;
    bool aux_skip_ones;
};
static int rs_run(const RsPlan& pl, const RsBuffers& b, uint64_t n, void* temp, hipStream_t s, const uint32_t* n_dev,
                  bool temp_zeroed, const uint32_t* ext_hist, bool exclusive, int key_shift = 0) {
    if (n == 0) return 0;
    if (n >= (1ull << 32)) { set_error("radix sort: more than 2^32-1 pairs"); return 1; }
    const bool scanned = rs_scanned(n);
    const RsTemp t = rs_carve(temp, n, pl, scanned);
    if (!temp_zeroed) MGS_HIP(zero_fill(t.hist, t.zero_bytes, s));
    const uint32_t tiles = rs_tiles(n, scanned);
    const int items = rs_tile_items(n, scanned);
    const bool payload = b.pa != nullptr;
    if (payload && !scanned) { set_error("radix sort: payloads need the counted-tiles path"); return 1; }
    const RsTree tree = rs_tree(tiles);
    RsTreeArgs ta;
    ta.levels = tree.levels;
    for (int l = 0; l < RS_MAX_LEVELS; ++l) ta.off[l] = l < tree.levels ? tree.off[l] : 0u;
    ta.top_rows = tree.rows[tree.levels - 1];
    if (!scanned && !ext_hist) {
        RsHistArgs h;
        h.npasses = pl.npasses; h.radix = pl.radix; h.sub = pl.sub; h.wide = pl.depth ? t.wide : nullptr;
        for (int p = 0; p < RS_MAX_PASSES; ++p) { h.shift[p] = pl.shift[p]; h.mask[p] = (1 << pl.db[p]) - 1; }
        hipLaunchKernelGGL(rs_hist_kernel, dim3(min(tiles, 1024u)), dim3(RS_THREADS), 0, s, b.ka, (uint32_t)n, n_dev, h, t.hist);
    }
    const uint32_t* ghist = (!scanned && ext_hist) ? ext_hist : t.hist;
    const int hstride = (!scanned && ext_hist) ? 256 : pl.radix;
    const uint32_t *kin = b.ka, *vin = b.va_is_index ? nullptr : b.va, *pin = b.pa;
    uint32_t *kout = b.kb, *vout = b.vb, *pout = b.pb;
    uint32_t *kalt = b.ka, *valt = b.va, *palt = b.pa;
    for (int p = 0; p < pl.npasses; ++p) {
        RsPassArgs a;
        a.kin = kin; a.vin = vin; a.pin = pin; a.kout = kout; a.vout = vout; a.pout = pout;
        a.n = (uint32_t)n; a.n_dev = n_dev; a.shift = pl.shift[p]; a.sub = pl.sub;
        a.hist = ghist + p * hstride;
        a.status = t.status + (size_t)p * rs_status_rows(tiles) * pl.radix;
        a.tiles = tiles;
        a.ticket = (exclusive && tiles <= 256u) ? nullptr : t.tickets + p;
        a.error = t.error;
        a.pass = p;
        a.xcd_band = (scanned && g_opt_radix_xcd_band != 0) ? 1 : 0;
        a.counts = t.counts; a.sums = t.sums + (size_t)p * tree.sum_rows * pl.radix;
        a.tree = ta;
        a.wide = pl.depth ? t.wide : nullptr;
        a.cond = pl.depth ? (p == 2 ? 1 : (p == 3 ? 2 : 0)) : 0;
        a.last = (!pl.depth && p == pl.npasses - 1) ? 1 : 0;
        a.vfinal = b.vfinal ? b.vfinal : vout;
        a.kfinal = b.vfinal ? b.kfinal : kout;
        a.ranges = (!pl.depth && p == pl.npasses - 1) ? b.ranges : nullptr;
        a.range_shift = key_shift;
        if (a.ranges && key_shift == 0) a.kfinal = nullptr;
        a.aux_in = b.aux_in; a.aux_out = b.aux_out; a.aux_skip_ones = b.aux_skip_ones ? 1 : 0;
        if (scanned) {
            RsTileHistArgs h;
            h.keys = kin; h.n = (uint32_t)n; h.n_dev = n_dev; h.shift = a.shift; h.sub = pl.sub; h.tiles = tiles; h.tr = ta;
            h.counts = t.counts; h.sums = const_cast<uint32_t*>(a.sums);
            h.wide = t.wide; h.detect = (pl.depth && p == 0) ? 1 : 0; h.only_if_wide = a.cond == 2 ? 1 : 0;
            if (items == RS_ITEMS_WIDE) {
                if (pl.db[p] == 9) rs_launch_tile_hist<RS_ITEMS_WIDE, 9>(h, s); else rs_launch_tile_hist<RS_ITEMS_WIDE, 8>(h, s);
            } else {
                if (pl.db[p] == 9) rs_launch_tile_hist<RS_ITEMS, 9>(h, s); else rs_launch_tile_hist<RS_ITEMS, 8>(h, s);
            }
        }
        const bool ballot = g_opt_radix_ballot_rank != 0;
        if (pl.db[p] == 9) {
            if (payload) rs_launch_pass_items<9, true>(a, items, scanned, tiles, ballot, s);
            else rs_launch_pass_items<9, false>(a, items, scanned, tiles, ballot, s);
        } else {
            if (payload) rs_launch_pass_items<8, true>(a, items, scanned, tiles, ballot, s);
            else rs_launch_pass_items<8, false>(a, items, scanned, tiles, ballot, s);
        }
        kin = kout; vin = vout; pin = pout;
        uint32_t* tk = kalt; kalt = kout; kout = tk;
        uint32_t* tv = valt; valt = vout; vout = tv;
        uint32_t* tp = palt; palt = pout; pout = tp;
    }
    MGS_HIP(hipGetLastError());
    return 0;
}

int radix_sort_pairs(uint32_t* ka, uint32_t* va, uint32_t* kb, uint32_t* vb, uint64_t n, int bits, void* temp,
                     hipStream_t s, const uint32_t* n_dev, bool temp_zeroed, const uint2* aux_in, uint2* aux_out,
                     const uint32_t* ext_hist, bool aux_empty_for_ones, bool exclusive, uint2* ranges, int key_shift) {
    RsPlan pl = rs_plan_plain(bits);
    for (int p = 0; p < RS_MAX_PASSES; ++p) pl.shift[p] += key_shift;
    if (pl.npasses > RS_MAX_PASSES) { set_error("radix sort: more than 32 key bits"); return 1; }
    RsBuffers b;
    b.ranges = ranges;
    b.ka = ka; b.va = va; b.va_is_index = false; b.pa = nullptr; b.kb = kb; b.vb = vb; b.pb = nullptr; b.kfinal = nullptr; b.vfinal = nullptr;
    b.aux_in = aux_in; b.aux_out = aux_out; b.aux_skip_ones = aux_empty_for_ones;
    return rs_run(pl, b, n, temp, s, n_dev, temp_zeroed, ext_hist, exclusive, key_shift);
}

int radix_sort_depth(uint32_t* keys, uint32_t* key_b, uint32_t* val_a, uint32_t* val_b, void* rect, bool payload,
                     uint32_t* perm, uint2* rect_sorted, uint64_t n, void* temp, hipStream_t s, bool temp_zeroed, bool exclusive) {
    const RsPlan pl = rs_plan_for_depth(n);
    RsBuffers b;
    b.ranges = nullptr;
    b.ka = keys; b.va = val_a; b.va_is_index = true; b.kb = key_b; b.vb = val_b;
    b.pa = payload ? (uint32_t*)rect : nullptr; b.pb = payload ? (uint32_t*)rect + n : nullptr;
    b.kfinal = nullptr; b.vfinal = perm;
    b.aux_in = payload ? nullptr : (const uint2*)rect; b.aux_out = rect_sorted; b.aux_skip_ones = true;
    return rs_run(pl, b, n, temp, s, nullptr, temp_zeroed, nullptr, exclusive);
}

int set_radix_spin_limit(uint32_t limit) {
    const uint32_t v = limit == 0xFFFFFFFFu ? RS_SPIN_LIMIT : limit;
    MGS_HIP(hipMemcpyToSymbol(HIP_SYMBOL(g_rs_spin_limit), &v, sizeof(v)));
    return 0;
}

}
```

Baseline: 2975 Mpix/s.

## Generate tile keys inside radix sort and move duplicate housekeeping into scan

Instead of having the duplicate kernel write (tile|depth, gaussian) pairs to memory, the first radix pass and its histogram now produce those keys on the fly. Each wave binary-searches the scanned offsets and expands rectangles into tile ids with DPP max-scans. The per-frame housekeeping that duplicate used to do (zeroing sort temp, resetting ranges and n_touched, writing count and status, rotating prepare) moves into the prefix-scan kernels, so the duplicate launch can be skipped entirely on the combined forward path. This trades the write and read of the duplicated key/value arrays for extra search and index arithmetic inside the sort's first pass, and it only applies to the non-ballot 8-bit-digit configuration.

```diff
diff --git a/monogs_amd/csrc/api.hip b/monogs_amd/csrc/api.hip
--- a/monogs_amd/csrc/api.hip
+++ b/monogs_amd/csrc/api.hip
@@ -1,4 +1,5 @@
 #include "common.h"
+#include "tile_gen.h"
 
 #include <stdarg.h>
 #include <stdio.h>
@@ -150,11 +151,13 @@
 }
 float* mgs_backward_tau(void* backward_scratch, int32_t P) { return backward_tau_out(backward_scratch, P < 0 ? 0 : P); }
 
-int mgs_forward_preprocess(const mgs_camera* cam, int32_t P, const float* means3D, const float* shs,
-                           const float* colors_precomp, const float* opacities, const float* scales,
-                           const float* rotations, const float* cov3D_precomp, void* geometry, int32_t* radii,
-                           void* prepare_backward, uint64_t* num_rendered, const uint32_t* prev_status,
-                           uint32_t* prev_status_out, mgs_timing* timing, void* stream) {
+}
+
+static int forward_preprocess_impl(const mgs_camera* cam, int32_t P, const float* means3D, const float* shs,
+                                   const float* colors_precomp, const float* opacities, const float* scales,
+                                   const float* rotations, const float* cov3D_precomp, void* geometry, int32_t* radii,
+                                   void* prepare_backward, uint64_t* num_rendered, const uint32_t* prev_status,
+                                   uint32_t* prev_status_out, mgs_timing* timing, void* stream, const ScanHousekeeping* hk) {
     if (check_cam(cam)) return 1;
     if (P < 0) { set_error("P must be >= 0"); return 1; }
     if (check_map_size(P)) return 1;
@@ -193,7 +196,7 @@
     const bool per_tile = binning_path(P, cam->image_width, cam->image_height) != 0;
     if (per_tile) {
         tm.mark();
-        if (int rc = launch_scan(g, P, s, exclusive, g.rect)) return rc;
+        if (int rc = launch_scan(g, P, s, exclusive, g.rect, hk)) return rc;
     } else {
         if (int rc = launch_depth_sort(g, P, depth_sort_payload(P, cam->image_width, cam->image_height), s, exclusive)) return rc;
         tm.mark();
@@ -220,11 +223,23 @@
     return 0;
 }
 
+extern "C" {
+
+int mgs_forward_preprocess(const mgs_camera* cam, int32_t P, const float* means3D, const float* shs,
+                           const float* colors_precomp, const float* opacities, const float* scales,
+                           const float* rotations, const float* cov3D_precomp, void* geometry, int32_t* radii,
+                           void* prepare_backward, uint64_t* num_rendered, const uint32_t* prev_status,
+                           uint32_t* prev_status_out, mgs_timing* timing, void* stream) {
+    return forward_preprocess_impl(cam, P, means3D, shs, colors_precomp, opacities, scales, rotations, cov3D_precomp, geometry,
+                                   radii, prepare_backward, num_rendered, prev_status, prev_status_out, timing, stream, nullptr);
+}
+
 static int g_opt_tile_sort_fused = 1;
 
 static int forward_render_impl(const mgs_camera* cam, int32_t P, uint64_t R, bool capacity, void* geometry,
                                void* binning, void* image, float* out_color, float* out_depth, float* out_opacity,
-                               int32_t* n_touched, uint32_t* overflow, mgs_timing* timing, void* stream) {
+                               int32_t* n_touched, uint32_t* overflow, mgs_timing* timing, void* stream,
+                               bool housekeeping_done = false) {
     if (check_cam(cam)) return 1;
     if (P < 0) { set_error("P must be >= 0"); return 1; }
     if (check_map_size(P)) return 1;
@@ -244,11 +259,14 @@
     if (cap) n_dev = b.count;
     const bool per_tile = binning_path(P, W, H) != 0;
     tm.mark();
-    if (int rc = launch_duplicate(*cam, P, g, b, capacity ? R : (R > 0 ? 0xFFFFFFFFull : 0ull), n_touched, img, R,
-                                  tile_bits(W, H), cap ? b.count : nullptr, overflow, s, per_tile)) return rc;
+    const bool generated = per_tile && R > 0 && radix_tile_sort_generated(R);
+    const TileGenArgs gen = generated ? tile_gen_args(*cam, P, g) : TileGenArgs{};
+    if (!(housekeeping_done && generated))
+        if (int rc = launch_duplicate(*cam, P, g, b, capacity ? R : (R > 0 ? 0xFFFFFFFFull : 0ull), n_touched, img, R,
+                                      tile_bits(W, H), cap ? b.count : nullptr, overflow, s, per_tile, !generated)) return rc;
     tm.mark();
     if (int rc = launch_sort(g, b, R, tile_bits(W, H), s, n_dev, (cam->flags & MGS_FLAG_EXCLUSIVE_DEVICE) != 0, img.ranges,
-                             per_tile)) return rc;
+                             per_tile, generated ? &gen : nullptr)) return rc;
     const uint32_t* sort_err = R > 0 ? radix_error_flag(b.sort_temp, R, tile_bits(W, H)) : nullptr;
     const bool sort_tiles = per_tile && R > 0;
     const TileSortArgs ts = sort_tiles ? tile_sort_args(*cam, g, b, R, n_dev) : TileSortArgs{};
@@ -271,6 +289,31 @@
     return 0;
 }
 
+}
+
+static bool forward_scan_housekeeping(const mgs_camera* cam, int32_t P, uint64_t capacity, void* geometry, void* binning,
+                                      void* image, int32_t* n_touched, uint32_t* status, ScanHousekeeping* hk) {
+    if (!cam || P <= 0 || capacity == 0 || capacity >= (1ull << 32) || !geometry || !binning || !image || !n_touched) return false;
+    if (check_cam(cam) || check_map_size(P)) return false;
+    const int W = cam->image_width, H = cam->image_height;
+    if (binning_path(P, W, H) == 0 || !radix_tile_sort_generated(capacity) || !scan_does_housekeeping(P)) return false;
+    const GeometryState g = GeometryState::carve(geometry, P);
+    const ImageState img = ImageState::carve(image, W, H);
+    const BinningState b = BinningState::carve(binning, capacity, W, H);
+    hk->n_touched = n_touched;
+    hk->ranges = img.ranges;
+    hk->ntiles = tiles_x(W) * tiles_y(H);
+    radix_zero_region(b.sort_temp, capacity, tile_bits(W, H), &hk->zero_ptr, &hk->zero_words);
+    hk->count = b.count;
+    hk->status = status;
+    hk->r_cap = (uint32_t)capacity;
+    hk->prepare = g.prepare;
+    hk->depth_err = radix_depth_error_flag(g.sort_temp, (uint64_t)P);
+    return true;
+}
+
+extern "C" {
+
 int mgs_forward_render(const mgs_camera* cam, int32_t P, uint64_t R, void* geometry, void* binning, void* image,
                        float* out_color, float* out_depth, float* out_opacity, int32_t* n_touched,
                        uint32_t* status, mgs_timing* timing, void* stream) {
@@ -291,10 +334,14 @@
                          const float* cov3D_precomp, void* geometry, int32_t* radii, void* prepare_backward,
                          uint64_t capacity, void* binning, void* image, float* out_color, float* out_depth,
                          float* out_opacity, int32_t* n_touched, uint32_t* overflow, mgs_timing* timing, void* stream) {
-    if (int rc = mgs_forward_preprocess(cam, P, means3D, shs, colors_precomp, opacities, scales, rotations, cov3D_precomp,
-                                        geometry, radii, prepare_backward, nullptr, nullptr, nullptr, timing, stream)) return rc;
-    return mgs_forward_render_capacity(cam, P, capacity, geometry, binning, image, out_color, out_depth, out_opacity,
-                                       n_touched, overflow, timing, stream);
+    ScanHousekeeping hk;
+    const bool moved = forward_scan_housekeeping(cam, P, capacity, geometry, binning, image, n_touched, overflow, &hk);
+    if (int rc = forward_preprocess_impl(cam, P, means3D, shs, colors_precomp, opacities, scales, rotations, cov3D_precomp,
+                                         geometry, radii, prepare_backward, nullptr, nullptr, nullptr, timing, stream,
+                                         moved ? &hk : nullptr)) return rc;
+    if (capacity == 0) { set_error("capacity must be > 0"); return 1; }
+    return forward_render_impl(cam, P, capacity, true, geometry, binning, image, out_color, out_depth, out_opacity, n_touched,
+                               overflow, timing, stream, moved);
 }
 
 int mgs_backward(const mgs_camera* cam, int32_t P, uint64_t R, const float* means3D, const float* shs,
@@ -434,6 +481,7 @@
     if (name && !strcmp(name, "radix_ballot_rank")) { g_opt_radix_ballot_rank = (int)value; return 0; }
     if (name && !strcmp(name, "radix_xcd_band")) { g_opt_radix_xcd_band = (int)value; return 0; }
     if (name && !strcmp(name, "debug_sort_exclusive")) { g_opt_debug_sort_exclusive = (int)value; return 0; }
+    if (name && !strcmp(name, "tile_sort_generated")) { g_opt_tile_sort_generated = value < 0 ? -1 : (int)value; return 0; }
     if (name && !strcmp(name, "dup_slot_major")) { g_opt_dup_slot_major = (int)value; return 0; }
     if (name && !strcmp(name, "blend_bwd_transposed")) {
         g_opt_blend_bwd_transposed = value < 0 ? 2 : (int)value;
diff --git a/monogs_amd/csrc/binning.hip b/monogs_amd/csrc/binning.hip
--- a/monogs_amd/csrc/binning.hip
+++ b/monogs_amd/csrc/binning.hip
@@ -1,5 +1,6 @@
 #include "common.h"
 #include "tile_sort.h"
+#include "tile_gen.h"
 
 
 namespace mgs {
@@ -48,22 +49,30 @@
     return total;
 }
 
+template <bool HK>
 __global__ void __launch_bounds__(SCAN_THREADS) scan_local_kernel(const uint2* __restrict__ rects, uint32_t* out,
-                                                                  uint32_t* block_sums, int n) {
+                                                                  uint32_t* block_sums, int n, ScanHousekeeping hk,
+                                                                  int n_threads ) {
     __shared__ uint32_t smem[8];
     const int lane = threadIdx.x & 63, wv = threadIdx.x >> 6;
     const int cbase = blockIdx.x * SCAN_ITEMS + wv * (SCAN_PER_THREAD * WAVE);
+    if constexpr (HK) {
+        grid_zero(hk.zero_ptr, hk.zero_words, (size_t)n_threads, SCAN_THREADS);
+        for (int j = blockIdx.x * SCAN_THREADS + threadIdx.x; j < hk.ntiles; j += n_threads) hk.ranges[j] = make_uint2(0xFFFFFFFFu, 0u);
+    }
     uint32_t incl[SCAN_PER_THREAD];
     const uint32_t total = scan_block_rows(rects, n, cbase, lane, wv, incl, smem);
 #pragma unroll
     for (int i = 0; i < SCAN_PER_THREAD; ++i) {
         const int idx = cbase + i * WAVE + lane;
         if (idx < n) out[idx] = incl[i];
+        if constexpr (HK) if (idx < n) hk.n_touched[idx] = 0;
     }
     if (threadIdx.x == 0) block_sums[blockIdx.x] = total;
 }
 
-__global__ void __launch_bounds__(SCAN_THREADS) scan_blocks_kernel(uint32_t* block_sums, int nblocks) {
+template <bool HK>
+__global__ void __launch_bounds__(SCAN_THREADS) scan_blocks_kernel(uint32_t* block_sums, int nblocks, ScanHousekeeping hk) {
     __shared__ uint32_t smem[8];
     uint32_t carry = 0;
     for (int start = 0; start < nblocks; start += SCAN_THREADS) {
@@ -75,6 +84,20 @@
         carry += total;
     }
     if (threadIdx.x == 0) block_sums[nblocks] = carry;
+    if constexpr (HK) {
+        if (threadIdx.x == 0) {
+            const bool depth_bad = hk.depth_err && radix_failed(hk.depth_err) != 0u;
+            const uint32_t R = depth_bad ? 0u : carry;
+            const uint32_t over = R > hk.r_cap ? 1u : 0u;
+            hk.count[0] = min(R, hk.r_cap);
+            hk.count[1] = over;
+            if (hk.status) hk.status[0] = over | (depth_bad ? (uint32_t)MGS_STATUS_DEPTH_SORT_TIMEOUT : 0u);
+            if (hk.prepare) {
+                hk.prepare[1] = hk.prepare[0];
+                hk.prepare[0] = 0ull;
+            }
+        }
+    }
 }
 
 constexpr uint32_t SCAN_SPIN_LIMIT = 1u << 22;
@@ -122,9 +145,10 @@
 }
 int g_opt_scan_small = -1;
 bool scan_is_small(int P) { return g_opt_scan_small != 0 && scan_nblocks(P) <= SCAN_SMALL_MAX_BLOCKS; }
-
-
-int launch_scan(const GeometryState& g, int P, hipStream_t s, bool exclusive, const uint2* rects) {
+bool scan_does_housekeeping(int P) { return P > 0 && !scan_is_small(P); }
+
+
+int launch_scan(const GeometryState& g, int P, hipStream_t s, bool exclusive, const uint2* rects, const ScanHousekeeping* hk) {
     if (P == 0) return 0;
     const int nb = scan_nblocks(P);
     if (scan_is_small(P)) {
@@ -134,23 +158,19 @@
         MGS_HIP(hipGetLastError());
         return 0;
     }
-    hipLaunchKernelGGL(scan_local_kernel, dim3(nb), dim3(SCAN_THREADS), 0, s, rects, g.point_offsets,
-                       g.scan_blocks, P);
-    hipLaunchKernelGGL(scan_blocks_kernel, dim3(1), dim3(SCAN_THREADS), 0, s, g.scan_blocks, nb);
+    if (hk) {
+        hipLaunchKernelGGL(scan_local_kernel<true>, dim3(nb), dim3(SCAN_THREADS), 0, s, rects, g.point_offsets, g.scan_blocks, P,
+                           *hk, nb * SCAN_THREADS);
+        hipLaunchKernelGGL(scan_blocks_kernel<true>, dim3(1), dim3(SCAN_THREADS), 0, s, g.scan_blocks, nb, *hk);
+    } else {
+        hipLaunchKernelGGL(scan_local_kernel<false>, dim3(nb), dim3(SCAN_THREADS), 0, s, rects, g.point_offsets, g.scan_blocks, P,
+                           ScanHousekeeping{}, nb * SCAN_THREADS);
+        hipLaunchKernelGGL(scan_blocks_kernel<false>, dim3(1), dim3(SCAN_THREADS), 0, s, g.scan_blocks, nb, ScanHousekeeping{});
+    }
     MGS_HIP(hipGetLastError());
     return 0;
 }
 
-__device__ __forceinline__ void dup_pair(uint32_t gidx, const uint32_t* __restrict__ depth_key, int lo, uint32_t& val,
-                                         uint32_t& kfield) {
-    val = gidx; kfield = 0u;
-    if (depth_key) {
-        const uint32_t k = depth_key[gidx];
-        const uint32_t d = k == 0xFFFFFFFFu ? DEPTH_KEY_NARROW : min(k - DEPTH_KEY_SUB, DEPTH_KEY_NARROW);
-        kfield = d >> lo;
-        if (lo) val |= (d & ((1u << lo) - 1u)) << (32 - lo);
-    }
-}
 __global__ void __launch_bounds__(256) duplicate_kernel(int P, const uint2* __restrict__ rects,
                                                         const uint32_t* __restrict__ perm,
                                                         const uint32_t* __restrict__ depth_key, int tshift, int lo,
@@ -164,7 +184,8 @@
                                                         const uint32_t* __restrict__ depth_err, int offsets_global,
                                                         uint32_t* __restrict__ hist , int hist_passes,
                                                         int n_threads , int slot_major,
-                                                        unsigned long long* __restrict__ prepare ) {
+                                                        unsigned long long* __restrict__ prepare ,
+                                                        int emit ) {
     const int i = blockIdx.x * 256 + threadIdx.x;
     if (i == 0 && prepare) {
         prepare[1] = prepare[0];
@@ -182,6 +203,7 @@
         overflow[0] = (count ? count[1] : 0u) | (depth_bad ? (uint32_t)MGS_STATUS_DEPTH_SORT_TIMEOUT : 0u);
     if (i < ntiles) ranges[i] = make_uint2(0xFFFFFFFFu, 0u);
     if (i < P) n_touched[i] = 0;
+    if (!emit) return;
     uint32_t idx = 0, nt = 0, off = 0, kf = 0;
     int x0 = 0, y0 = 0, x1 = 0;
     if (i < P) {
@@ -350,12 +372,12 @@
 
 int launch_duplicate(const mgs_camera& cam, int P, const GeometryState& g, const BinningState& b, uint64_t r_cap,
                      int32_t* n_touched, const ImageState& img, uint64_t sort_n, int sort_bits, uint32_t* count,
-                     uint32_t* overflow, hipStream_t s, bool per_tile) {
+                     uint32_t* overflow, hipStream_t s, bool per_tile, bool emit) {
     const uint32_t* depth_err = P > 0 ? radix_depth_error_flag(g.sort_temp, (uint64_t)P) : nullptr;
     const int ntiles = tiles_x(cam.image_width) * tiles_y(cam.image_height);
     int n = P > ntiles ? P : ntiles;
     if (n == 0) return 0;
-    const bool slot_major = P > 0 && g_opt_dup_slot_major != 0 &&
+    const bool slot_major = emit && P > 0 && g_opt_dup_slot_major != 0 &&
                             (g_opt_dup_slot_major > 0 || (sort_n >= DUP_SLOT_MAJOR_MIN && sort_n >= 6ull * (uint64_t)P));
     if (slot_major) {
         const uint64_t want = sort_n / 8;
@@ -375,7 +397,7 @@
                        zero_words, count, overflow, depth_err,
                        (P > 0 && scan_is_small(P)) ? 1 : 0,
                        count_digits ? g.tile_hist : nullptr, (sort_bits + 7) / 8, n_threads, slot_major ? 1 : 0,
-                       P > 0 ? g.prepare : nullptr);
+                       P > 0 ? g.prepare : nullptr, emit ? 1 : 0);
     MGS_HIP(hipGetLastError());
     return 0;
 }
@@ -387,12 +409,21 @@
                             g.sort_temp, s, true, exclusive);
 }
 
+TileGenArgs tile_gen_args(const mgs_camera& cam, int P, const GeometryState& g) {
+    const int tb = tile_bits(cam.image_width, cam.image_height);
+    TileGenArgs ga;
+    ga.rects = g.rect; ga.depth_key = g.depth_key; ga.offsets = g.point_offsets; ga.block_sums = g.scan_blocks;
+    ga.P = P; ga.gx = tiles_x(cam.image_width); ga.tshift = 32 - tb; ga.lo = tile_depth_lo_bits(tb);
+    ga.offsets_global = (P > 0 && scan_is_small(P)) ? 1 : 0;
+    return ga;
+}
+
 int launch_sort(const GeometryState& g, const BinningState& b, uint64_t R, int bits, hipStream_t s, const uint32_t* n_dev,
-                bool exclusive, uint2* ranges, bool per_tile) {
+                bool exclusive, uint2* ranges, bool per_tile, const TileGenArgs* gen) {
     if (R == 0) return 0;
     const bool counted = bits <= 16 && radix_wants_hist(R) && g.tile_hist != nullptr;
     return radix_sort_pairs(b.keys_a, b.vals_a, b.keys_b, b.vals_b, R, bits, b.sort_temp, s, n_dev, true, nullptr, nullptr,
-                            counted ? g.tile_hist : nullptr, false, exclusive, ranges, per_tile ? 32 - bits : 0);
+                            counted ? g.tile_hist : nullptr, false, exclusive, ranges, per_tile ? 32 - bits : 0, gen);
 }
 
 TileSortArgs tile_sort_args(const mgs_camera& cam, const GeometryState& g, const BinningState& b, uint64_t R,
diff --git a/monogs_amd/csrc/common.h b/monogs_amd/csrc/common.h
--- a/monogs_amd/csrc/common.h
+++ b/monogs_amd/csrc/common.h
@@ -176,10 +176,24 @@
 inline float* backward_grad_acc(void* scratch) { return (float*)align_up((size_t)scratch, 256); }
 inline float* backward_tau_part(void* scratch, int P) { return backward_grad_acc(scratch) + (size_t)P * GRAD_FLOATS; }
 inline float* backward_tau_out(void* scratch, int P) { return backward_tau_part(scratch, P) + (size_t)TAU_SLOTS * 16; }
-int launch_scan(const GeometryState& g, int P, hipStream_t s, bool exclusive, const uint2* rects);
+struct ScanHousekeeping {
+    int32_t* n_touched;
+    uint2* ranges;
+    int ntiles;
+    uint32_t* zero_ptr;
+    size_t zero_words;
+    uint32_t* count;
+    uint32_t* status;
+    uint32_t r_cap;
+    unsigned long long* prepare;
+    const uint32_t* depth_err;
+};
+bool scan_does_housekeeping(int P);
+int launch_scan(const GeometryState& g, int P, hipStream_t s, bool exclusive, const uint2* rects,
+                const ScanHousekeeping* hk = nullptr);
 int launch_duplicate(const mgs_camera& cam, int P, const GeometryState& g, const BinningState& b, uint64_t r_cap,
                      int32_t* n_touched, const ImageState& img, uint64_t sort_n, int sort_bits, uint32_t* count,
-                     uint32_t* overflow, hipStream_t s, bool per_tile);
+                     uint32_t* overflow, hipStream_t s, bool per_tile, bool emit = true);
 size_t sort_temp_bytes(uint64_t n, int bits);
 size_t radix_temp_bytes(uint64_t n, int bits);
 size_t radix_depth_temp_bytes(uint64_t n);
@@ -190,6 +204,7 @@
 __device__ __forceinline__ uint32_t radix_failed(const uint32_t* __restrict__ e) { return (e[0] | e[1]) | (e[2] | e[3]); }
 void radix_zero_region(void* temp, uint64_t n, int bits, uint32_t** ptr, size_t* words);
 void radix_depth_zero_region(void* temp, uint64_t n, uint32_t** ptr, size_t* words, bool header_only = false);
+struct TileGenArgs;
 int radix_sort_pairs(uint32_t* ka, uint32_t* va, uint32_t* kb, uint32_t* vb, uint64_t n, int bits, void* temp,
                      hipStream_t s, const uint32_t* n_dev = nullptr, bool temp_zeroed = false,
                      const uint2* aux_in = nullptr, uint2* aux_out = nullptr,
@@ -197,7 +212,9 @@
                      bool aux_empty_for_ones = false,
                      bool exclusive = false,
                      uint2* ranges = nullptr,
-                     int key_shift = 0);
+                     int key_shift = 0,
+                     const TileGenArgs* gen = nullptr);
+bool radix_tile_sort_generated(uint64_t n);
 bool radix_wants_hist(uint64_t n);
 bool radix_depth_payload(uint64_t n);
 int radix_sort_depth(uint32_t* keys, uint32_t* key_b, uint32_t* val_a, uint32_t* val_b, void* rect, bool payload,
@@ -206,7 +223,8 @@
 inline bool depth_sort_payload(int P, int W, int H) { return radix_depth_payload((uint64_t)P) && tiles_x(W) <= 255 && tiles_y(H) <= 255; }
 int launch_depth_sort(const GeometryState& g, int P, bool payload, hipStream_t s, bool exclusive = false);
 int launch_sort(const GeometryState& g, const BinningState& b, uint64_t R, int bits, hipStream_t s,
-                const uint32_t* n_dev = nullptr, bool exclusive = false, uint2* ranges = nullptr, bool per_tile = false);
+                const uint32_t* n_dev = nullptr, bool exclusive = false, uint2* ranges = nullptr, bool per_tile = false,
+                const TileGenArgs* gen = nullptr);
 struct TileSortArgs {
     uint32_t* keys;
     uint32_t* vals;
@@ -224,7 +242,7 @@
 int set_radix_spin_limit(uint32_t limit);
 extern bool g_opt_blend_bwd_transposed_set;
 extern int g_dbg_last_bwd_split;
-extern int g_opt_radix_ballot_rank, g_opt_radix_scanned, g_opt_radix_xcd_band, g_opt_knn_grid_min, g_opt_scan_small, g_opt_dup_slot_major, g_opt_blend_bwd_transposed, g_opt_blend_bwd_split, g_opt_blend_bwd_split_min, g_opt_blend_bwd_split_frac;
+extern int g_opt_tile_sort_generated, g_opt_radix_ballot_rank, g_opt_radix_scanned, g_opt_radix_xcd_band, g_opt_knn_grid_min, g_opt_scan_small, g_opt_dup_slot_major, g_opt_blend_bwd_transposed, g_opt_blend_bwd_split, g_opt_blend_bwd_split_min, g_opt_blend_bwd_split_frac;
 int launch_blend_forward(const mgs_camera& cam, const GeometryState& g, const BinningState& b,
                          const ImageState& img, float* out_color, float* out_depth, float* out_opacity,
                          int32_t* n_touched, const uint32_t* sort_err, uint32_t* status, const TileSortArgs* tile_sort,
diff --git a/monogs_amd/csrc/radix_sort.hip b/monogs_amd/csrc/radix_sort.hip
--- a/monogs_amd/csrc/radix_sort.hip
+++ b/monogs_amd/csrc/radix_sort.hip
@@ -1,4 +1,5 @@
 #include "common.h"
+#include "tile_gen.h"
 
 namespace mgs {
 
@@ -40,10 +41,16 @@
 int g_opt_radix_scanned = -1;
 int g_opt_radix_ballot_rank = 0;
 int g_opt_radix_xcd_band = 1;
+int g_opt_tile_sort_generated = -1;
 constexpr uint64_t RS_SCANNED_MIN = 64ull * 1024;
 static inline bool rs_scanned(uint64_t n) {
     if (g_opt_radix_scanned >= 0) return g_opt_radix_scanned == 1 && n > RS_SCANNED_MIN;
     return n > RS_ONE_SWEEP_MAX;
+}
+
+bool radix_tile_sort_generated(uint64_t n) {
+    if (g_opt_tile_sort_generated == 0 || g_opt_radix_ballot_rank != 0 || !rs_scanned(n)) return false;
+    return g_opt_tile_sort_generated > 0 || n > RS_ONE_SWEEP_MAX;
 }
 
 int binning_path(int P, int W, int H) {
@@ -208,8 +215,9 @@
     uint32_t* wide;
     int detect;
     int only_if_wide;
+    TileGenArgs gen;
 };
-template <int ITEMS, int TPW, int DB>
+template <int ITEMS, int TPW, int DB, bool GEN = false>
 __global__ void __launch_bounds__(RS_THREADS * TPW) rs_tile_hist_kernel(RsTileHistArgs a) {
     static_assert(TPW == 1 || TPW == (1 << RS_FAN_LOG), "a workgroup counts one tile or one level-1 node");
     constexpr int RADIX = 1 << DB, DPT = RADIX / RS_THREADS, COPIES = 16 / DPT;
@@ -223,10 +231,19 @@
     const uint32_t tile = blockIdx.x * TPW + q, tile_start = tile * TILE_PAIRS;
     const uint32_t tile_n = tile_start < n_live ? min(TILE_PAIRS, n_live - tile_start) : 0u;
     uint32_t k[ITEMS];
-#pragma unroll
-    for (int i = 0; i < ITEMS; ++i) {
-        const uint32_t e = (uint32_t)i * RS_THREADS + t;
-        k[i] = e < tile_n ? a.keys[tile_start + e] : 0xFFFFFFFFu;
+    if constexpr (GEN) {
+        static_assert(RS_WAVES * TILE_GEN_LDS_WORDS <= COPIES * RADIX, "the generator's scratch lives in the counters");
+        uint32_t unused[1];
+        const uint32_t s0 = tile_start + (uint32_t)wv * (ITEMS * WAVE);
+        tile_gen_wave<ITEMS, false>(a.gen, tile_n ? s0 : 0u, tile_n ? tile_start + tile_n : 0u,
+                                    &wh[q][0][0] + wv * TILE_GEN_LDS_WORDS, lane, k, unused);
+        __syncthreads();
+    } else {
+#pragma unroll
+        for (int i = 0; i < ITEMS; ++i) {
+            const uint32_t e = (uint32_t)i * RS_THREADS + t;
+            k[i] = e < tile_n ? a.keys[tile_start + e] : 0xFFFFFFFFu;
+        }
     }
 #pragma unroll
     for (int i = 0; i < COPIES; ++i)
@@ -241,7 +258,8 @@
     for (int i = 0; i < ITEMS; ++i) {
         const uint32_t x = rs_xf(k[i], a.sub);
         far |= k[i] != 0xFFFFFFFFu && x >= RS_DEPTH_NARROW;
-        if ((uint32_t)i * RS_THREADS + t < tile_n) atomicAdd(&mine[(x >> a.shift) & (RADIX - 1)], 1u);
+        const uint32_t e = GEN ? (uint32_t)wv * (ITEMS * WAVE) + (uint32_t)i * WAVE + lane : (uint32_t)i * RS_THREADS + t;
+        if (e < tile_n) atomicAdd(&mine[(x >> a.shift) & (RADIX - 1)], 1u);
     }
     if (a.detect && far) atomicOr(a.wide, 1u);
     __syncthreads();
@@ -281,12 +299,12 @@
     RS_DRAIN();
     RS_HSTAMP(3);
 }
-template <int ITEMS, int DB>
+template <int ITEMS, int DB, bool GEN = false>
 static void rs_launch_tile_hist(const RsTileHistArgs& a, hipStream_t s) {
     if (a.tiles >= 1024u)
-        hipLaunchKernelGGL((rs_tile_hist_kernel<ITEMS, 4, DB>), dim3((a.tiles + 3) / 4), dim3(RS_THREADS * 4), 0, s, a);
+        hipLaunchKernelGGL((rs_tile_hist_kernel<ITEMS, 4, DB, GEN>), dim3((a.tiles + 3) / 4), dim3(RS_THREADS * 4), 0, s, a);
     else
-        hipLaunchKernelGGL((rs_tile_hist_kernel<ITEMS, 1, DB>), dim3(a.tiles), dim3(RS_THREADS), 0, s, a);
+        hipLaunchKernelGGL((rs_tile_hist_kernel<ITEMS, 1, DB, GEN>), dim3(a.tiles), dim3(RS_THREADS), 0, s, a);
 }
 
 struct RsPassArgs {
@@ -320,6 +338,7 @@
     const uint32_t* counts;
     const uint32_t* sums;
     RsTreeArgs tree;
+    TileGenArgs gen;
 };
 
 template <int ITEMS>
@@ -375,7 +394,12 @@
     return true;
 }
 
-template <int ITEMS, int DB, bool SCANNED, bool PAYLOAD, bool BALLOT, bool VIDX>
+template <bool GEN, int RADIX>
+__device__ __forceinline__ uint32_t rs_digit(uint32_t k, const RsPassArgs& a) {
+    return GEN ? (k >> a.shift) & (RADIX - 1) : (rs_xf(k, a.sub) >> a.shift) & (RADIX - 1);
+}
+
+template <int ITEMS, int DB, bool SCANNED, bool PAYLOAD, bool BALLOT, bool VIDX, bool GEN = false>
 __global__ void __launch_bounds__(RS_THREADS, (SCANNED && ITEMS == RS_ITEMS_WIDE && DB == 8 && !PAYLOAD) ? 7 : 1) rs_pass_kernel(RsPassArgs a) {
     constexpr int TILE_PAIRS = RS_THREADS * ITEMS;
     constexpr int RADIX = 1 << DB, DPT = RADIX / RS_THREADS;
@@ -386,6 +410,8 @@
     __shared__ uint32_t sbuf[SBUF];
     __shared__ uint32_t wsum[RS_WAVES];
     __shared__ uint32_t s_tile;
+    constexpr int STASH = (GEN && ITEMS == RS_ITEMS_WIDE) ? 3 : 0;
+    __shared__ uint32_t s_stash[STASH ? STASH * RS_THREADS : 1];
 
     const int t = threadIdx.x, lane = t & 63, wv = t >> 6;
     const bool wide = a.wide ? a.wide[0] != 0u : false;
@@ -416,7 +442,8 @@
     if (tile == 0xFFFFFFFFu) return;
     const uint32_t tile_start = tile * (uint32_t)TILE_PAIRS;
     if (tile_start >= n_live) return;
-    const uint32_t tile_n = min((uint32_t)TILE_PAIRS, n_live - tile_start);
+    const uint32_t tile_n = GEN ? (uint32_t)__builtin_amdgcn_readfirstlane((int)min((uint32_t)TILE_PAIRS, n_live - tile_start))
+                                : min((uint32_t)TILE_PAIRS, n_live - tile_start);
 
     uint32_t hcount[DPT], before[DPT];
 #pragma unroll
@@ -425,77 +452,95 @@
     uint4 lv[RS_MAX_LEVELS - 1][DPT], tv[RS_TOP_BATCH / RS_WAVES][DPT];
     uint32_t lw[RS_MAX_LEVELS - 1], tw[RS_TOP_BATCH / RS_WAVES], tb[RS_TOP_BATCH / RS_WAVES];
     const int levels = a.tree.levels;
-    const uint32_t top_node = tile >> (RS_FAN_LOG * (levels - 1));
+    const uint32_t rtile = GEN ? (uint32_t)__builtin_amdgcn_readfirstlane((int)tile) : tile;
+    const uint32_t rw = GEN ? (uint32_t)__builtin_amdgcn_readfirstlane(wv) : (uint32_t)wv;
+    const uint32_t top_node = rtile >> (RS_FAN_LOG * (levels - 1));
     const uint4* __restrict__ c4 = reinterpret_cast<const uint4*>(a.counts);
     const uint4* __restrict__ top4 = levels == 1 ? c4 : reinterpret_cast<const uint4*>(a.sums) + (size_t)a.tree.off[levels - 1] * R4;
-    if (SCANNED) {
-#pragma unroll
-        for (int l = 0; l < RS_MAX_LEVELS - 1; ++l) {
-            const bool have = l < levels - 1;
-            const uint32_t node = tile >> (RS_FAN_LOG * l), first = node & ~3u, nb = node & 3u;
-            const uint4* base = (l == 0 || !have) ? c4 : reinterpret_cast<const uint4*>(a.sums) + (size_t)a.tree.off[l] * R4;
-            lw[l] = (have && (uint32_t)wv < nb) ? 1u : 0u;
-#pragma unroll
-            for (int j = 0; j < DPT; ++j) lv[l][j] = base[(size_t)(lw[l] ? first + (uint32_t)wv : 0u) * R4 + j * WAVE + lane];
-        }
-#pragma unroll
-        for (int q = 0; q < RS_TOP_BATCH / RS_WAVES; ++q) {
-            const uint32_t r = (uint32_t)wv + 4u * q;
-            tw[q] = r < a.tree.top_rows ? 1u : 0u;
-            tb[q] = r < top_node ? 1u : 0u;
-#pragma unroll
-            for (int j = 0; j < DPT; ++j) tv[q][j] = top4[(size_t)(tw[q] ? r : 0u) * R4 + j * WAVE + lane];
-        }
+    auto request_rows = [&]() {
+        if (SCANNED) {
+#pragma unroll
+            for (int l = 0; l < RS_MAX_LEVELS - 1; ++l) {
+                const bool have = l < levels - 1;
+                const uint32_t node = rtile >> (RS_FAN_LOG * l), first = node & ~3u, nb = node & 3u;
+                const uint4* base = (l == 0 || !have) ? c4 : reinterpret_cast<const uint4*>(a.sums) + (size_t)a.tree.off[l] * R4;
+                lw[l] = (have && rw < nb) ? 1u : 0u;
+#pragma unroll
+                for (int j = 0; j < DPT; ++j) lv[l][j] = base[(size_t)(lw[l] ? first + rw : 0u) * R4 + j * WAVE + lane];
+            }
+#pragma unroll
+            for (int q = 0; q < RS_TOP_BATCH / RS_WAVES; ++q) {
+                const uint32_t r = rw + 4u * q;
+                tw[q] = r < a.tree.top_rows ? 1u : 0u;
+                tb[q] = r < top_node ? 1u : 0u;
+#pragma unroll
+                for (int j = 0; j < DPT; ++j) tv[q][j] = top4[(size_t)(tw[q] ? r : 0u) * R4 + j * WAVE + lane];
+            }
+        } else {
+#pragma unroll
+            for (int j = 0; j < DPT; ++j) hcount[j] = a.hist[t * DPT + j];
+        }
+    };
+    if constexpr (!GEN) request_rows();
+
+    uint32_t key[ITEMS], val[ITEMS], rank[ITEMS], pay[PAYLOAD ? ITEMS : 1];
+    if constexpr (GEN) {
+        static_assert(SCANNED && !PAYLOAD && !VIDX && TILE_GEN_LDS_WORDS <= 2 * RADIX, "scratch = the wave's rows of `part` below");
+        tile_gen_wave<ITEMS, true>(a.gen, tile_start + (uint32_t)wv * (ITEMS * WAVE), tile_start + tile_n,
+                                   sbuf + wv * 2 * RADIX, lane, key, val);
+        __builtin_amdgcn_wave_barrier();
+#pragma unroll
+        for (int k = 0; k < STASH; ++k) s_stash[k * RS_THREADS + t] = val[ITEMS - 1 - k];
     } else {
 #pragma unroll
-        for (int j = 0; j < DPT; ++j) hcount[j] = a.hist[t * DPT + j];
-    }
-
-    uint32_t key[ITEMS], val[ITEMS], rank[ITEMS], pay[PAYLOAD ? ITEMS : 1];
-#pragma unroll
-    for (int i = 0; i < ITEMS; ++i) {
-        const uint32_t e = (uint32_t)wv * (ITEMS * WAVE) + (uint32_t)i * WAVE + lane;
-        const bool valid = e < tile_n;
-        key[i] = valid ? a.kin[tile_start + e] : 0xFFFFFFFFu;
-        if constexpr (VIDX) val[i] = tile_start + e;
-        else val[i] = valid ? a.vin[tile_start + e] : 0u;
-        if constexpr (PAYLOAD) pay[i] = valid ? a.pin[tile_start + e] : 0u;
-    }
-    if (SCANNED) {
-        uint4* part = reinterpret_cast<uint4*>(sbuf);
-#pragma unroll
-        for (int j = 0; j < DPT; ++j) {
-            uint4 ab = make_uint4(0u, 0u, 0u, 0u), at = make_uint4(0u, 0u, 0u, 0u);
-#pragma unroll
-            for (int l = 0; l < RS_MAX_LEVELS - 1; ++l) {
-                ab.x += lw[l] ? lv[l][j].x : 0u; ab.y += lw[l] ? lv[l][j].y : 0u; ab.z += lw[l] ? lv[l][j].z : 0u; ab.w += lw[l] ? lv[l][j].w : 0u;
-            }
-#pragma unroll
-            for (int q = 0; q < RS_TOP_BATCH / RS_WAVES; ++q) {
-                at.x += tw[q] ? tv[q][j].x : 0u; at.y += tw[q] ? tv[q][j].y : 0u; at.z += tw[q] ? tv[q][j].z : 0u; at.w += tw[q] ? tv[q][j].w : 0u;
-                ab.x += tb[q] ? tv[q][j].x : 0u; ab.y += tb[q] ? tv[q][j].y : 0u; ab.z += tb[q] ? tv[q][j].z : 0u; ab.w += tb[q] ? tv[q][j].w : 0u;
-            }
-            for (uint32_t r0 = RS_TOP_BATCH; r0 < a.tree.top_rows; r0 += RS_TOP_BATCH)
+        for (int i = 0; i < ITEMS; ++i) {
+            const uint32_t e = (uint32_t)wv * (ITEMS * WAVE) + (uint32_t)i * WAVE + lane;
+            const bool valid = e < tile_n;
+            key[i] = valid ? a.kin[tile_start + e] : 0xFFFFFFFFu;
+            if constexpr (VIDX) val[i] = tile_start + e;
+            else val[i] = valid ? a.vin[tile_start + e] : 0u;
+            if constexpr (PAYLOAD) pay[i] = valid ? a.pin[tile_start + e] : 0u;
+        }
+    }
+    auto sum_rows = [&]() {
+        if (SCANNED) {
+            uint4* part = reinterpret_cast<uint4*>(sbuf);
+#pragma unroll
+            for (int j = 0; j < DPT; ++j) {
+                uint4 ab = make_uint4(0u, 0u, 0u, 0u), at = make_uint4(0u, 0u, 0u, 0u);
+#pragma unroll
+                for (int l = 0; l < RS_MAX_LEVELS - 1; ++l) {
+                    ab.x += lw[l] ? lv[l][j].x : 0u; ab.y += lw[l] ? lv[l][j].y : 0u; ab.z += lw[l] ? lv[l][j].z : 0u; ab.w += lw[l] ? lv[l][j].w : 0u;
+                }
 #pragma unroll
                 for (int q = 0; q < RS_TOP_BATCH / RS_WAVES; ++q) {
-                    const uint32_t r = r0 + (uint32_t)wv + 4u * q;
-                    if (r < a.tree.top_rows) {
-                        const uint4 v = top4[(size_t)r * R4 + j * WAVE + lane];
-                        at.x += v.x; at.y += v.y; at.z += v.z; at.w += v.w;
-                        if (r < top_node) { ab.x += v.x; ab.y += v.y; ab.z += v.z; ab.w += v.w; }
+                    at.x += tw[q] ? tv[q][j].x : 0u; at.y += tw[q] ? tv[q][j].y : 0u; at.z += tw[q] ? tv[q][j].z : 0u; at.w += tw[q] ? tv[q][j].w : 0u;
+                    ab.x += tb[q] ? tv[q][j].x : 0u; ab.y += tb[q] ? tv[q][j].y : 0u; ab.z += tb[q] ? tv[q][j].z : 0u; ab.w += tb[q] ? tv[q][j].w : 0u;
+                }
+                for (uint32_t r0 = RS_TOP_BATCH; r0 < a.tree.top_rows; r0 += RS_TOP_BATCH)
+#pragma unroll
+                    for (int q = 0; q < RS_TOP_BATCH / RS_WAVES; ++q) {
+                        const uint32_t r = r0 + rw + 4u * q;
+                        if (r < a.tree.top_rows) {
+                            const uint4 v = top4[(size_t)r * R4 + j * WAVE + lane];
+                            at.x += v.x; at.y += v.y; at.z += v.z; at.w += v.w;
+                            if (r < top_node) { ab.x += v.x; ab.y += v.y; ab.z += v.z; ab.w += v.w; }
+                        }
                     }
-                }
-            part[(wv * 2 + 0) * R4 + j * WAVE + lane] = ab;
-            part[(wv * 2 + 1) * R4 + j * WAVE + lane] = at;
-        }
-    }
+                part[(rw * 2 + 0) * R4 + j * WAVE + lane] = ab;
+                part[(rw * 2 + 1) * R4 + j * WAVE + lane] = at;
+            }
+        }
+    };
+    if constexpr (GEN) request_rows();
+    sum_rows();
     RS_DRAIN();
     RS_STAMP(1);
     if (!BALLOT) {
 #pragma unroll
         for (int i = 0; i < ITEMS; ++i) {
             const uint32_t e = (uint32_t)wv * (ITEMS * WAVE) + (uint32_t)i * WAVE + lane;
-            const uint32_t d = (rs_xf(key[i], a.sub) >> a.shift) & (RADIX - 1);
+            const uint32_t d = rs_digit<GEN, RADIX>(key[i], a);
             rank[i] = 0;
             if (e < tile_n) rank[i] = __hip_atomic_fetch_add(&wave_hist[wv][d], 1u, __ATOMIC_RELAXED, __HIP_MEMORY_SCOPE_WORKGROUP);
         }
@@ -505,7 +550,7 @@
         for (int i = 0; i < ITEMS; ++i) {
             const uint32_t e = (uint32_t)wv * (ITEMS * WAVE) + (uint32_t)i * WAVE + lane;
             const bool valid = e < tile_n;
-            const uint32_t d = (rs_xf(key[i], a.sub) >> a.shift) & (RADIX - 1);
+            const uint32_t d = rs_digit<GEN, RADIX>(key[i], a);
             unsigned long long peers = __builtin_amdgcn_ballot_w64(valid);
 #pragma unroll
             for (int b = 0; b < DB; ++b) {
@@ -587,11 +632,13 @@
 #pragma unroll
     for (int i = 0; i < ITEMS; ++i) {
         const uint32_t e = (uint32_t)wv * (ITEMS * WAVE) + (uint32_t)i * WAVE + lane;
-        const uint32_t d = (rs_xf(key[i], a.sub) >> a.shift) & (RADIX - 1);
+        const uint32_t d = rs_digit<GEN, RADIX>(key[i], a);
         rank[i] = e < tile_n ? digit_base[d] + wave_hist[wv][d] + rank[i] : 0xFFFFFFFFu;
     }
     rs_exchange<ITEMS>(sbuf, rank, key, t);
     __syncthreads();
+#pragma unroll
+    for (int k = 0; k < STASH; ++k) val[ITEMS - 1 - k] = s_stash[k * RS_THREADS + t];
     rs_exchange<ITEMS>(sbuf, rank, val, t);
     if constexpr (PAYLOAD) {
         __syncthreads();
@@ -604,7 +651,7 @@
     for (int i = 0; i < ITEMS; ++i) {
         const uint32_t p = (uint32_t)i * RS_THREADS + t;
         live[i] = p < tile_n;
-        g[i] = gbase[(rs_xf(key[i], a.sub) >> a.shift) & (RADIX - 1)] + p;
+        g[i] = gbase[rs_digit<GEN, RADIX>(key[i], a)] + p;
     }
     if (!final_pass) {
 #pragma unroll
@@ -639,7 +686,7 @@
             if (p < tile_n && (p == 0 || lr != kr)) {
                 atomicMin(&a.ranges[kr].x, g[i]);
                 if (p > 0)
-                    atomicMax(&a.ranges[lr].y, gbase[(rs_xf(l, a.sub) >> a.shift) & (RADIX - 1)] + p);
+                    atomicMax(&a.ranges[lr].y, gbase[rs_digit<GEN, RADIX>(l, a)] + p);
             }
             if (p + 1 == tile_n) atomicMax(&a.ranges[kr].y, g[i] + 1u);
         }
@@ -697,7 +744,13 @@
 bool radix_depth_payload(uint64_t n) { return n > 0 && rs_scanned(n); }
 
 template <int ITEMS, int DB, bool SCANNED, bool PAYLOAD>
-static void rs_launch_pass(const RsPassArgs& a, uint32_t tiles, bool ballot, hipStream_t s) {
+static void rs_launch_pass(const RsPassArgs& a, uint32_t tiles, bool ballot, hipStream_t s, bool gen = false) {
+    if constexpr (SCANNED && DB == 8 && !PAYLOAD) {
+        if (gen) {
+            hipLaunchKernelGGL((rs_pass_kernel<ITEMS, 8, true, false, false, false, true>), dim3(tiles), dim3(RS_THREADS), 0, s, a);
+            return;
+        }
+    }
     if (ballot && DB == 8 && !PAYLOAD && a.vin != nullptr)
         hipLaunchKernelGGL((rs_pass_kernel<ITEMS, 8, SCANNED, false, true, false>), dim3(tiles), dim3(RS_THREADS), 0, s, a);
     else if (a.vin == nullptr && (DB == 9 || !SCANNED))
@@ -706,10 +759,11 @@
         hipLaunchKernelGGL((rs_pass_kernel<ITEMS, DB, SCANNED, PAYLOAD, false, false>), dim3(tiles), dim3(RS_THREADS), 0, s, a);
 }
 template <int DB, bool PAYLOAD>
-static void rs_launch_pass_items(const RsPassArgs& a, int items, bool scanned, uint32_t tiles, bool ballot, hipStream_t s) {
+static void rs_launch_pass_items(const RsPassArgs& a, int items, bool scanned, uint32_t tiles, bool ballot, hipStream_t s,
+                                 bool gen = false) {
     if (scanned) {
-        if (items == RS_ITEMS_WIDE) rs_launch_pass<RS_ITEMS_WIDE, DB, true, PAYLOAD>(a, tiles, ballot, s);
-        else rs_launch_pass<RS_ITEMS, DB, true, PAYLOAD>(a, tiles, ballot, s);
+        if (items == RS_ITEMS_WIDE) rs_launch_pass<RS_ITEMS_WIDE, DB, true, PAYLOAD>(a, tiles, ballot, s, gen);
+        else rs_launch_pass<RS_ITEMS, DB, true, PAYLOAD>(a, tiles, ballot, s, gen);
     } else if constexpr (!PAYLOAD && DB == 8) {
         if (items == RS_ITEMS_SMALL) rs_launch_pass<RS_ITEMS_SMALL, 8, false, false>(a, tiles, ballot, s);
         else if (items == RS_ITEMS_MID) rs_launch_pass<RS_ITEMS_MID, 8, false, false>(a, tiles, ballot, s);
@@ -728,7 +782,8 @@
     bool aux_skip_ones;
 };
 static int rs_run(const RsPlan& pl, const RsBuffers& b, uint64_t n, void* temp, hipStream_t s, const uint32_t* n_dev,
-                  bool temp_zeroed, const uint32_t* ext_hist, bool exclusive, int key_shift = 0) {
+                  bool temp_zeroed, const uint32_t* ext_hist, bool exclusive, int key_shift = 0,
+                  const TileGenArgs* gen_args = nullptr) {
     if (n == 0) return 0;
     if (n >= (1ull << 32)) { set_error("radix sort: more than 2^32-1 pairs"); return 1; }
     const bool scanned = rs_scanned(n);
@@ -776,24 +831,29 @@
         a.range_shift = key_shift;
         if (a.ranges && key_shift == 0) a.kfinal = nullptr;
         a.aux_in = b.aux_in; a.aux_out = b.aux_out; a.aux_skip_ones = b.aux_skip_ones ? 1 : 0;
+        const bool ballot = g_opt_radix_ballot_rank != 0;
+        const bool gen = gen_args && p == 0 && scanned && !ballot && !payload && !pl.depth && pl.db[0] == 8;
+        a.gen = gen ? *gen_args : TileGenArgs{};
         if (scanned) {
             RsTileHistArgs h;
+            h.gen = a.gen;
             h.keys = kin; h.n = (uint32_t)n; h.n_dev = n_dev; h.shift = a.shift; h.sub = pl.sub; h.tiles = tiles; h.tr = ta;
             h.counts = t.counts; h.sums = const_cast<uint32_t*>(a.sums);
             h.wide = t.wide; h.detect = (pl.depth && p == 0) ? 1 : 0; h.only_if_wide = a.cond == 2 ? 1 : 0;
-            if (items == RS_ITEMS_WIDE) {
+            if (gen) {
+                if (items == RS_ITEMS_WIDE) rs_launch_tile_hist<RS_ITEMS_WIDE, 8, true>(h, s); else rs_launch_tile_hist<RS_ITEMS, 8, true>(h, s);
+            } else if (items == RS_ITEMS_WIDE) {
                 if (pl.db[p] == 9) rs_launch_tile_hist<RS_ITEMS_WIDE, 9>(h, s); else rs_launch_tile_hist<RS_ITEMS_WIDE, 8>(h, s);
             } else {
                 if (pl.db[p] == 9) rs_launch_tile_hist<RS_ITEMS, 9>(h, s); else rs_launch_tile_hist<RS_ITEMS, 8>(h, s);
             }
         }
-        const bool ballot = g_opt_radix_ballot_rank != 0;
         if (pl.db[p] == 9) {
             if (payload) rs_launch_pass_items<9, true>(a, items, scanned, tiles, ballot, s);
             else rs_launch_pass_items<9, false>(a, items, scanned, tiles, ballot, s);
         } else {
             if (payload) rs_launch_pass_items<8, true>(a, items, scanned, tiles, ballot, s);
-            else rs_launch_pass_items<8, false>(a, items, scanned, tiles, ballot, s);
+            else rs_launch_pass_items<8, false>(a, items, scanned, tiles, ballot, s, gen);
         }
         kin = kout; vin = vout; pin = pout;
         uint32_t* tk = kalt; kalt = kout; kout = tk;
@@ -806,7 +866,8 @@
 
 int radix_sort_pairs(uint32_t* ka, uint32_t* va, uint32_t* kb, uint32_t* vb, uint64_t n, int bits, void* temp,
                      hipStream_t s, const uint32_t* n_dev, bool temp_zeroed, const uint2* aux_in, uint2* aux_out,
-                     const uint32_t* ext_hist, bool aux_empty_for_ones, bool exclusive, uint2* ranges, int key_shift) {
+                     const uint32_t* ext_hist, bool aux_empty_for_ones, bool exclusive, uint2* ranges, int key_shift,
+                     const TileGenArgs* gen) {
     RsPlan pl = rs_plan_plain(bits);
     for (int p = 0; p < RS_MAX_PASSES; ++p) pl.shift[p] += key_shift;
     if (pl.npasses > RS_MAX_PASSES) { set_error("radix sort: more than 32 key bits"); return 1; }
@@ -814,7 +875,7 @@
     b.ranges = ranges;
     b.ka = ka; b.va = va; b.va_is_index = false; b.pa = nullptr; b.kb = kb; b.vb = vb; b.pb = nullptr; b.kfinal = nullptr; b.vfinal = nullptr;
     b.aux_in = aux_in; b.aux_out = aux_out; b.aux_skip_ones = aux_empty_for_ones;
-    return rs_run(pl, b, n, temp, s, n_dev, temp_zeroed, ext_hist, exclusive, key_shift);
+    return rs_run(pl, b, n, temp, s, n_dev, temp_zeroed, ext_hist, exclusive, key_shift, gen);
 }
 
 int radix_sort_depth(uint32_t* keys, uint32_t* key_b, uint32_t* val_a, uint32_t* val_b, void* rect, bool payload,
diff --git a/monogs_amd/csrc/tile_gen.h b/monogs_amd/csrc/tile_gen.h
--- /dev/null
+++ b/monogs_amd/csrc/tile_gen.h
@@ -0,0 +1,120 @@
+#pragma once
+#include "common.h"
+
+namespace mgs {
+
+__device__ __forceinline__ void dup_pair(uint32_t gidx, const uint32_t* __restrict__ depth_key, int lo, uint32_t& val,
+                                         uint32_t& kfield) {
+    val = gidx; kfield = 0u;
+    if (depth_key) {
+        const uint32_t k = depth_key[gidx];
+        const uint32_t d = k == 0xFFFFFFFFu ? DEPTH_KEY_NARROW : min(k - DEPTH_KEY_SUB, DEPTH_KEY_NARROW);
+        kfield = d >> lo;
+        if (lo) val |= (d & ((1u << lo) - 1u)) << (32 - lo);
+    }
+}
+
+struct TileGenArgs {
+    const uint2* rects;
+    const uint32_t* depth_key;
+    const uint32_t* offsets;
+    const uint32_t* block_sums;
+    int P, gx, tshift, lo, offsets_global;
+};
+TileGenArgs tile_gen_args(const mgs_camera& cam, int P, const GeometryState& g);
+constexpr int TILE_GEN_LDS_WORDS = 6 * WAVE;
+
+template <int ITEMS, bool FULL>
+__device__ __forceinline__ void tile_gen_wave(const TileGenArgs& a, uint32_t s0_, uint32_t s1_, uint32_t* __restrict__ lds,
+                                              int lane, uint32_t (&key)[ITEMS], uint32_t (&val)[FULL ? ITEMS : 1]) {
+    uint32_t *s_own = lds, *s_off = lds + WAVE, *s_xy = lds + 2 * WAVE, *s_w = lds + 3 * WAVE, *s_kf = lds + 4 * WAVE,
+             *s_idx = lds + 5 * WAVE;
+#pragma unroll
+    for (int i = 0; i < ITEMS; ++i) key[i] = 0xFFFFFFFFu;
+#pragma unroll
+    for (int i = 0; i < (FULL ? ITEMS : 1); ++i) val[i] = 0u;
+    const uint32_t s0 = (uint32_t)__builtin_amdgcn_readfirstlane((int)s0_), s1 = (uint32_t)__builtin_amdgcn_readfirstlane((int)s1_);
+    if (s0 >= s1) return;
+    const uint32_t P = (uint32_t)a.P;
+    auto incl = [&](uint32_t k) { return a.offsets[k] + (a.offsets_global ? 0u : a.block_sums[k / SCAN_ITEMS]); };
+    uint32_t g;
+    {
+        uint32_t lo = 0, hi = P;
+        while (hi - lo > 1u) {
+            const uint32_t span = hi - lo, step = (span + 63u) / 64u;
+            const uint32_t probe = lo + min(((uint32_t)lane + 1u) * step, span) - 1u;
+            const unsigned long long above = __builtin_amdgcn_ballot_w64(incl(probe) > s0);
+            const int k = above ? __builtin_ctzll(above) : 63;
+            const uint32_t pk = lo + min(((uint32_t)k + 1u) * step, span) - 1u;
+            const uint32_t pk1 = k == 0 ? lo : lo + min((uint32_t)k * step, span);
+            lo = pk1; hi = pk + 1u;
+        }
+        g = lo;
+    }
+    uint32_t Eg = 0, exc = 0, carry = 0;
+    auto load_group = [&](uint32_t cb) {
+        const uint32_t gi = g + (uint32_t)lane;
+        const bool valid = gi < P;
+        uint32_t inc = 0, idg = 0, kfg = 0, xy = 0;
+        int gw = 1;
+        uint32_t ntg = 0;
+        if (valid) {
+            inc = incl(gi);
+            const uint2 r = a.rects[gi];
+            gw = (int)(r.y & 0xFFFFu);
+            ntg = (uint32_t)(gw * (int)(r.y >> 16));
+            xy = r.x;
+            if (FULL) dup_pair(gi, a.depth_key, a.lo, idg, kfg);
+        }
+        exc = ntg ? inc - ntg : 0xFFFFFFFFu;
+        const int last = (int)min(63u, P - 1u - g);
+        Eg = (uint32_t)__builtin_amdgcn_readlane((int)inc, last);
+        __builtin_amdgcn_wave_barrier();
+        s_off[lane] = exc; s_xy[lane] = xy; s_w[lane] = (uint32_t)max(gw, 1);
+        if (FULL) { s_idx[lane] = idg; s_kf[lane] = kfg; }
+        const unsigned long long before = __builtin_amdgcn_ballot_w64(exc < cb);
+        carry = before ? 64u - (uint32_t)__builtin_clzll(before) : 0u;
+    };
+    load_group(s0);
+    uint32_t sl = s0;
+#pragma unroll
+    for (int i = 0; i < ITEMS; ++i) {
+        const uint32_t cb = s0 + (uint32_t)i * WAVE;
+        const uint32_t ce = min(cb + (uint32_t)WAVE, s1);
+        while (sl < ce) {
+            const uint32_t e = min(ce, Eg);
+            if (e > sl) {
+                __builtin_amdgcn_wave_barrier();
+                s_own[lane] = 0u;
+                __builtin_amdgcn_wave_barrier();
+                if (exc - cb < (uint32_t)WAVE) s_own[exc - cb] = (uint32_t)lane + 1u;
+                __builtin_amdgcn_wave_barrier();
+                uint32_t m = s_own[lane];
+#define MGS_DPP_MAX(ctrl, row_mask) m = max(m, (uint32_t)__builtin_amdgcn_update_dpp(0, (int)m, ctrl, row_mask, 0xf, false))
+                MGS_DPP_MAX(0x111, 0xf); MGS_DPP_MAX(0x112, 0xf); MGS_DPP_MAX(0x114, 0xf); MGS_DPP_MAX(0x118, 0xf);
+                MGS_DPP_MAX(0x142, 0xa); MGS_DPP_MAX(0x143, 0xc);
+#undef MGS_DPP_MAX
+                const uint32_t owner = max(m, carry);
+                carry = (uint32_t)__builtin_amdgcn_readlane((int)owner, 63);
+                const uint32_t o = cb + (uint32_t)lane;
+                if (owner != 0u && o >= sl && o < e) {
+                    const uint32_t L = owner - 1u;
+                    const uint32_t t = o - s_off[L];
+                    const uint32_t w = s_w[L], xy = s_xy[L];
+                    const uint32_t yy = t / w, xx = t - yy * w;
+                    const uint32_t tid = ((xy >> 16) + yy) * (uint32_t)a.gx + (xy & 0xFFFFu) + xx;
+                    key[i] = tid << a.tshift;
+                    if (FULL) { key[i] |= s_kf[L]; val[i] = s_idx[L]; }
+                }
+                sl = e;
+            }
+            if (sl < ce) {
+                g += WAVE;
+                if (g >= P) { sl = s1; break; }
+                load_group(cb);
+            }
+        }
+    }
+}
+
+}
```

Result: slower. 2936 Mpix/s (-1.3%).
